# tatsuya-ogawa/GaussianSplattingMlx

Hardware: AMD Instinct MI355X
Metric: train views/sec (full step: fwd + L1/DSSIM loss + bwd + Adam + densify/prune at the reference cadence), Lego 800x800 300k Gaussians (higher is better)
Workload: dtype f32

## Files before the change

### gaussiansplattingmlx_amd/_lib.py

```python
from __future__ import annotations

import ctypes as C
import os

HERE = os.path.dirname(os.path.abspath(__file__))
LIB_PATH = os.environ.get("GSPLAT_LIB", os.path.join(HERE, "libgsplat_hip.so"))

GS_OK = 0
STATUS = {1: "GS_ERR_INVALID_ARG", 2: "GS_ERR_SIZE_MISMATCH", 3: "GS_ERR_WORKSPACE_OVERFLOW", 4: "GS_ERR_HIP",
          5: "GS_ERR_NO_FORWARD", 6: "GS_ERR_NO_DEVICE", 7: "GS_ERR_IO", 8: "GS_ERR_COMM", 9: "GS_ERR_REPLICA_MISMATCH"}
GS_ERR_REPLICA_MISMATCH = 9


class GsplatError(RuntimeError):
    def __init__(self, code, msg):
        super().__init__(f"{STATUS.get(code, code)}: {msg}")
        self.code = code


class gs_camera(C.Structure):
    _fields_ = [("view", C.c_float * 16), ("proj", C.c_float * 16), ("cam_center", C.c_float * 3),
                ("fov_x", C.c_float), ("fov_y", C.c_float), ("focal_x", C.c_float), ("focal_y", C.c_float)]


# ... 26 lines not shown

class gs_adc_params(C.Structure):
    _fields_ = [(n, C.c_float) for n in ("grad_threshold", "percent_dense", "min_opacity", "max_screen_size", "prune_world",
                                         "scene_extent")]


GS_DEPTH_ACCUMULATED, GS_DEPTH_EXPECTED, GS_DEPTH_DISPARITY = 0, 1, 2
GS_DP_ALLREDUCE, GS_DP_SH_COMPRESSED = 0, 1
GS_DP_UNIQUE_ID_BYTES = 128

_vp = C.c_void_p
_SIGS = {
    "gs_dp_unique_id": (C.c_int, [_vp]),
    "gs_dp_init": (C.c_int, [_vp, _vp, C.c_int, C.c_int]),
    "gs_dp_attach": (C.c_int, [_vp, _vp, C.c_int, C.c_int]),
    "gs_dp_shutdown": (C.c_int, [_vp]),
    "gs_dp_info": (C.c_int, [_vp, C.POINTER(C.c_int), C.POINTER(C.c_int)]),
    "gs_dp_step": (C.c_int, [_vp, C.c_int, C.POINTER(gs_dp_step_args)]),
    "gs_dp_allreduce_sum": (C.c_int, [_vp, _vp, C.c_longlong]),
    "gs_dp_check_overflow": (C.c_int, [_vp, C.POINTER(C.c_int), C.POINTER(C.c_longlong)]),
    "gs_dp_exchange_timing": (C.c_int, [_vp, C.c_int]),
    "gs_dp_exchange_read": (C.c_int, [_vp, _vp, C.POINTER(C.c_int), C.POINTER(C.c_int)]),
    "gs_abi_version": (C.c_int, []),
    "gs_ctx_create": (C.c_int, [C.c_int] * 7 + [C.POINTER(_vp)]),
    "gs_ctx_destroy": (C.c_int, [_vp]),
    "gs_ctx_set_stream": (C.c_int, [_vp, _vp]),
    "gs_ctx_reserve": (C.c_int, [_vp, C.c_int, C.c_longlong]),
    "gs_workspace_bytes": (C.c_size_t, [_vp]),
    "gs_sync": (C.c_int, [_vp]),
    "gs_overflow_pending": (C.c_int, [_vp, C.POINTER(C.c_uint32)]),
    "gs_wait": (C.c_int, [_vp]),
    "gs_last_error": (C.c_char_p, [_vp]),
    "gs_projection_forward": (C.c_int, [_vp, C.c_int, C.c_int] + [_vp] * 4 + [C.POINTER(gs_camera)] + [_vp] * 8),
    "gs_projection_backward": (C.c_int, [_vp, C.c_int, C.c_int] + [_vp] * 4 + [C.POINTER(gs_camera)] + [_vp] * 10),
    "gs_tile_bin": (C.c_int, [_vp, C.c_int] + [_vp] * 4),
    "gs_tile_bin_cut": (C.c_int, [_vp, C.c_int] + [_vp] * 5),
    "gs_tile_bin_info": (C.c_int, [_vp, C.POINTER(C.c_uint32), C.POINTER(C.c_uint32)]),
    "gs_tile_bin_views": (C.c_int, [_vp, C.POINTER(_vp), C.POINTER(_vp), C.POINTER(_vp)]),
    "gs_tile_bin_export": (C.c_int, [_vp, _vp, _vp, _vp]),
    "gs_build_packed_tile_indices": (C.c_int, [_vp, C.c_uint32, _vp]),
    "gs_pack_gaussians": (C.c_int, [_vp, C.c_int] + [_vp] * 6),
    "gs_blend_forward": (C.c_int, [_vp, C.c_int] + [_vp] * 5),
    "gs_blend_backward": (C.c_int, [_vp, C.c_int] + [_vp] * 9),
    "gs_blend_contrib": (C.c_int, [_vp, C.c_int] + [_vp] * 3),
    "gs_render_contrib": (C.c_int, [_vp, _vp, _vp]),
    "gs_contrib_actions": (C.c_int, [_vp, C.c_int, _vp, C.c_float, _vp, _vp]),
    "gs_ssim_window": (C.c_int, [C.c_int, C.c_float, _vp]),
    "gs_ssim_forward": (C.c_int, [_vp] + [C.c_int] * 4 + [_vp] * 9),
    "gs_ssim_backward": (C.c_int, [_vp] + [C.c_int] * 4 + [_vp] * 11),
    "gs_render_forward": (C.c_int, [_vp, C.c_int, C.c_int] + [_vp] * 6 + [C.POINTER(gs_camera)] + [_vp] * 4),
    "gs_render_backward": (C.c_int, [_vp] + [_vp] * 9),
    "gs_render_backward_dp": (C.c_int, [_vp] + [_vp] * 8),
    "gs_render_backward_adam": (C.c_int, [_vp] * 7 + [C.c_longlong, _vp, C.c_float, C.c_float, C.c_float, C.c_float]),
    "gs_render_backward_dp_begin": (C.c_int, [_vp] * 5),
    "gs_render_backward_dp_finish": (C.c_int, [_vp] * 5),
    "gs_render_backward_dp_finish_geom": (C.c_int, [_vp] * 6),
    "gs_render_backward_dp_geom": (C.c_int, [_vp] * 10),
    "gs_sh_grad_from_views_adam_dir": (C.c_int, [_vp, C.c_int, C.c_int, C.c_int] + [_vp] * 9 + [C.c_longlong] + [C.c_float] * 6 + [_vp]),
    "gs_adam_step_add": (C.c_int, [_vp, C.c_longlong] + [_vp] * 4 + [C.c_int, _vp, _vp] + [C.c_float] * 4 + [_vp, C.c_longlong]),
    "gs_sh_grad_from_views": (C.c_int, [_vp, C.c_int, C.c_int, C.c_int] + [_vp] * 5),
    "gs_accum_grad_norm": (C.c_int, [_vp, C.c_int, _vp, _vp, _vp]),
    "gs_classify_gaussians": (C.c_int, [_vp, C.c_int, _vp, C.c_float, _vp, C.c_int, _vp, C.c_float, C.c_float,
                                        C.c_float, C.c_int, _vp, _vp]),
    "gs_densify_offsets": (C.c_int, [_vp, C.c_int, _vp, _vp, _vp, _vp]),
    "gs_build_densify_output_map": (C.c_int, [_vp, C.c_int, _vp, _vp, C.c_int, _vp, _vp]),
    "gs_densify_gather": (C.c_int, [_vp, C.c_int, C.c_int] + [_vp] * 15),
    "gs_densify_plan": (C.c_int, [_vp, C.c_int, _vp, _vp, _vp]),
    "gs_densify_plan_read": (C.c_int, [_vp, C.c_int, _vp, C.POINTER(C.c_int)]),
    "gs_build_densify_output_map_planned": (C.c_int, [_vp, C.c_int, _vp, _vp, C.c_int, _vp, _vp]),
    "gs_densify_gather_planned": (C.c_int, [_vp, C.c_int, C.c_int] + [_vp] * 8 + [C.c_ulonglong] + [_vp] * 6),
    "gs_densify_gather_planned_packed": (C.c_int, [_vp, C.c_int, C.c_int] + [_vp] * 8 + [C.c_ulonglong, _vp, C.POINTER(C.c_int)]),
    "gs_densify_noise": (C.c_int, [_vp, C.c_ulonglong, C.c_int, _vp]),
    "gs_ply_write": (C.c_int, [_vp, C.c_char_p, C.c_int, C.c_int] + [_vp] * 6),
    "gs_ply_probe": (C.c_int, [_vp, C.c_char_p, _vp, _vp, _vp]),
    "gs_ply_load": (C.c_int, [_vp, C.c_char_p, C.c_int, C.c_int] + [_vp] * 6),
    "gs_ply_pack_rows": (C.c_int, [_vp, C.c_int, C.c_int] + [_vp] * 7),
    "gs_set_block_work_buffer": (C.c_int, [_vp, _vp]),
    "gs_view_hint_words": (C.c_int, [_vp, C.POINTER(C.c_int)]),
    "gs_set_view_hints": (C.c_int, [_vp, _vp, C.c_int]),
    "gs_set_depth_cuts": (C.c_int, [_vp, C.c_int]),
    "gs_clear_depth_cuts": (C.c_int, [_vp, _vp, C.c_int]),
    "gs_forward_missed": (C.c_int, [_vp, C.POINTER(C.c_int)]),
    "gs_cut_stats": (C.c_int, [_vp, C.POINTER(C.c_uint32)]),
    "gs_set_grad_norm_accum": (C.c_int, [_vp, _vp]),
    "gs_block_count": (C.c_int, [_vp, _vp]),
    "gs_copy_block_work": (C.c_int, [_vp, _vp]),
    "gs_dist_topk": (C.c_int, [_vp, C.c_int, C.c_int, C.c_int, C.c_int, _vp, _vp]),
    "gs_sh_grad_from_views_adam": (C.c_int, [_vp, C.c_int, C.c_int, C.c_int] + [_vp] * 8 + [C.c_longlong] + [C.c_float] * 6),
    "gs_loss_target_cache_floats": (C.c_int, [_vp, C.POINTER(C.c_longlong)]),
    "gs_set_loss_target_cache": (C.c_int, [_vp, _vp, C.c_int]),
    "gs_set_loss_mask": (C.c_int, [_vp, _vp]),
    "gs_loss_forward_backward": (C.c_int, [_vp] + [_vp] * 5 + [C.c_float, C.c_float] + [_vp] * 3),
    "gs_depth_loss": (C.c_int, [_vp, C.POINTER(gs_depth_loss_params)] + [_vp] * 7),
    "gs_depth_normalize": (C.c_int, [_vp, C.c_longlong, _vp, _vp, C.c_float, _vp]),
    "gs_image_metrics": (C.c_int, [_vp, C.c_int, C.c_int] + [_vp] * 4),
    "gs_colour_moments": (C.c_int, [_vp, C.c_longlong] + [_vp] * 4),
    "gs_adam_step": (C.c_int, [_vp, C.c_longlong] + [_vp] * 4 + [C.c_int, _vp, _vp] + [C.c_float] * 4),
    "gs_profile_enable": (C.c_int, [_vp, C.c_uint]),
    "gs_profile_read": (C.c_int, [_vp, _vp, _vp]),
    "gs_copy_last_contrib": (C.c_int, [_vp, _vp]),
    "gs_last_stats": (C.c_int, [_vp, C.POINTER(C.c_uint32)]),
    "gs_ctx_set_tuning": (C.c_int, [_vp, C.c_int, C.c_longlong]),
    "gs_copy_overflow_flag": (C.c_int, [_vp, _vp]),
    "gs_set_update_gate": (C.c_int, [_vp, _vp]),
    "gs_set_overflow_rider": (C.c_int, [_vp, _vp]),
    "gs_set_pose_correction": (C.c_int, [_vp, _vp, _vp]),
# ... 11 lines not shown
    "gs_get_absgrad": (C.c_int, [_vp, C.c_int, _vp]),
    "gs_set_adc_stats": (C.c_int, [_vp, _vp, _vp, _vp]),
    "gs_adc_accumulate": (C.c_int, [_vp, C.c_int, _vp, _vp, C.c_int, _vp, _vp, _vp]),
    "gs_adc_classify": (C.c_int, [_vp, C.c_int] + [_vp] * 4 + [C.c_int, _vp, C.POINTER(gs_adc_params), C.c_int, C.c_int, _vp, _vp]),
    "gs_adc_gather": (C.c_int, [_vp, C.c_int, C.c_int] + [_vp] * 9 + [C.c_int] + [_vp] * 6),
    "gs_adc_gather_moments": (C.c_int, [_vp, C.c_int, C.c_int, _vp, _vp, _vp, C.POINTER(_vp), C.POINTER(_vp)]),
    "gs_adc_reset_opacity": (C.c_int, [_vp, C.c_int, _vp, _vp, _vp, C.c_float]),
    "gs_set_sparse_adam": (C.c_int, [_vp, C.c_int]),
    "gs_get_visibility": (C.c_int, [_vp, C.c_int, _vp]),
    "gs_adam_step_visible": (C.c_int, [_vp, C.c_longlong] + [_vp] * 4 + [C.c_int, _vp, _vp, _vp] + [C.c_float] * 4 + [C.c_int, _vp]),
    "gs_set_filter3d_cameras": (C.c_int, [_vp, C.c_int, _vp]),
    "gs_compute_filter3d": (C.c_int, [_vp, C.c_int, _vp, _vp]),
    "gs_set_filter3d": (C.c_int, [_vp, _vp]),
    "gs_filter3d_bake": (C.c_int, [_vp, C.c_int] + [_vp] * 5),
    "gs_undistort": (C.c_int, [_vp, C.POINTER(gs_lens)] + [C.c_int] * 6 + [_vp, _vp, _vp]),
    "gs_undistort_fisheye": (C.c_int, [_vp, C.POINTER(gs_fisheye_lens)] + [C.c_int] * 6 + [_vp, _vp, _vp]),
    "gs_set_mcmc": (C.c_int, [_vp, _vp]),
    "gs_mcmc_regularizer_grad": (C.c_int, [_vp, C.c_int] + [_vp] * 5),
    "gs_mcmc_inject_noise": (C.c_int, [_vp, C.c_int] + [_vp] * 4 + [C.c_float, _vp]),
    "gs_mcmc_random": (C.c_int, [_vp, C.c_ulonglong, C.c_int, C.c_int, C.c_int, _vp, _vp, _vp]),
    "gs_mcmc_relocate": (C.c_int, [_vp, C.c_int, C.c_int] + [_vp] * 11),
    "gs_mcmc_grow": (C.c_int, [_vp, C.c_int, C.c_int, C.c_int] + [_vp] * 11),
    "gs_set_gathered_gate": (C.c_int, [_vp, C.c_longlong, C.c_int, _vp]),
    "gs_set_gate_seen": (C.c_int, [_vp, _vp]),
    "gs_dp_cc_floats": (C.c_longlong, [C.c_int]),
    "gs_dp_check_replicas": (C.c_int, [_vp, C.c_int, _vp, C.c_longlong]),
    "gs_dp_check_replicas_begin": (C.c_int, [_vp, C.c_int, _vp, C.c_longlong]),
    "gs_dp_check_replicas_end": (C.c_int, [_vp]),
    "gs_dp_check_plan": (C.c_int, [_vp, C.POINTER(C.c_longlong), C.c_int]),
}

_lib = None


def load():
    global _lib
    if _lib is not None:
        return _lib
    if not os.path.exists(LIB_PATH):
        raise ImportError(f"{LIB_PATH} is missing: run `python -m gaussiansplattingmlx_amd.build` "
                          "(or __graft_entry__.build()). There is no CPU fallback.")
    import torch
    lib = C.CDLL(LIB_PATH)
    for name, (res, args) in _SIGS.items():
        fn = getattr(lib, name)
        fn.restype = res
        fn.argtypes = args
    _lib = lib
    return lib


TUNE_FWD_WAVES_PER_SIMD, TUNE_BWD_WAVES_PER_CU, TUNE_FWD_QUADRANTS, TUNE_OP_FWD_PPL, TUNE_OP_BWD_PPL, \
    TUNE_FWD_TRACE_BUFFER, TUNE_DEPTH_GRADIENT, TUNE_WIDE_TILE_SORT, TUNE_HOST_OVERFLOW_ERRORS, TUNE_SPLITTER_DEPTH_SORT, \
    TUNE_COLOUR_RIDERS, TUNE_FWD_QUEUES, TUNE_FWD_FOUR_WAVES, TUNE_FWD_FOLD_TEST_SCALE, TUNE_POISON_CHECKPOINTS, TUNE_RENDER_ONLY, TUNE_FWD_PAIR, TUNE_FWD_SLOW_SLOT, TUNE_TRIM_RECTS = range(19)


def exported_symbols():
    return list(_SIGS)


def make_camera(view, proj, camCenter, fovX, fovY, focalX, focalY) -> gs_camera:
    import numpy as np
    cam = gs_camera()
    v = np.asarray(view, dtype=np.float32).reshape(16)
    p = np.asarray(proj, dtype=np.float32).reshape(16)
    cc = np.asarray(camCenter, dtype=np.float32).reshape(3)
    for i in range(16):
        cam.view[i] = float(v[i])
        cam.proj[i] = float(p[i])
    for i in range(3):
        cam.cam_center[i] = float(cc[i])
    cam.fov_x, cam.fov_y, cam.focal_x, cam.focal_y = float(fovX), float(fovY), float(focalX), float(focalY)
    return cam
```

### gaussiansplattingmlx_amd/csrc/api.hip

```cpp
#include <math.h>
#include <stdlib.h>
#include <stdio.h>
#include <string.h>

#include "gs_ctx.h"
#include <vector>

using namespace gs;

namespace {

int fail(gs_ctx* c, int code, const std::string& msg)
{
    if (c) c->err = msg;
    return code;
}

template <class T>
int dev_alloc(gs_ctx* c, T** p, size_t count)
{
    *p = nullptr;
    if (count == 0) count = 1;
    GS_HIP_CHECK(c, hipMalloc((void**)p, count * sizeof(T)));
    c->ws_bytes += count * sizeof(T);
    return GS_OK;
}

template <class T>
void dev_free(T*& p)
{
    if (p) (void)hipFree(p);
    p = nullptr;
}

void free_gaussian_ws(gs_ctx* c)
{
    dev_free(c->packed12); dev_free(c->gradAcc16);
    dev_free(c->depthKey[0]); dev_free(c->depthKey[1]); dev_free(c->depthVal[0]); dev_free(c->depthVal[1]);
    dev_free(c->tilesTouched); dev_free(c->tileRect); dev_free(c->tilePieces); dev_free(c->waveSeg); dev_free(c->scanPrefix); dev_free(c->scanTmp); dev_free(c->blockSums);
    dev_free(c->visPerBlock); dev_free(c->dropPerBlock);
    dev_free(c->bucketId);
    dev_free(c->densifyTiles);
    c->densifyTileCap = 0;
}

void free_pair_ws(gs_ctx* c)
{
    dev_free(c->pairKey[0]); dev_free(c->pairKey[1]); dev_free(c->pairVal[0]); dev_free(c->pairVal[1]);
    dev_free(c->segSlot); dev_free(c->itemBlock); dev_free(c->itemRow);
}

int ensure_arena(gs_ctx* c)
{
    if (!c->fast16 || c->capM <= 0) return GS_OK;
    long long want = (c->pairsReserved || c->reserving) ? c->capM / 80 : c->segCap * 4;
    if (want < 65536) want = 65536;
    if (want > c->segCap * 4) want = c->segCap * 4;
    if (want < c->qslotWanted) want = c->qslotWanted;
    if (want <= c->qslotCap) return GS_OK;
    GS_HIP_CHECK(c, hipStreamSynchronize(c->stream));
    if (c->segState) { c->ws_bytes -= (size_t)c->qslotCap * 5 * 64 * sizeof(float); dev_free(c->segState); }
    const int rc = dev_alloc(c, &c->segState, (size_t)want * 5 * 64);
    if (rc) { c->qslotCap = 0; return rc; }
    c->qslotCap = want;
    c->fwd.valid = false;
    return GS_OK;
}

int ensure_capacity(gs_ctx* c, int N, long long M)
{
    bool grewN = false, grewM = false;
    if (N > c->capN) {
        GS_HIP_CHECK(c, hipStreamSynchronize(c->stream));
        free_gaussian_ws(c);
        const size_t n = (size_t)N;
        int rc;
        if ((rc = dev_alloc(c, &c->packed12, n * 12))) return rc;
        if ((rc = dev_alloc(c, &c->gradAcc16, n * 16))) return rc;
        for (int i = 0; i < 2; i++) {
            if ((rc = dev_alloc(c, &c->depthKey[i], n))) return rc;
            if ((rc = dev_alloc(c, &c->depthVal[i], n))) return rc;
        }
        if ((rc = dev_alloc(c, &c->tilesTouched, n))) return rc;
        if ((rc = dev_alloc(c, &c->tileRect, n))) return rc;
        if ((rc = dev_alloc(c, &c->tilePieces, n))) return rc;
        if ((rc = dev_alloc(c, &c->waveSeg, (n / 64 + 8) * GS_EXPAND_SLICES))) return rc;
        if ((rc = dev_alloc(c, &c->scanPrefix, (n / 64 + 16) * GS_EXPAND_SLICES))) return rc;
        if ((rc = dev_alloc(c, &c->scanTmp, (n / 64 + 16) * GS_EXPAND_SLICES / 1024 + 8))) return rc;
        const size_t nb = n / GS_SCAN_BLOCK + 2;
        if ((rc = dev_alloc(c, &c->blockSums, nb))) return rc;
        if ((rc = dev_alloc(c, &c->visPerBlock, n / 128 + 2))) return rc;
        dev_free(c->dropPerBlock);
        if ((rc = dev_alloc(c, &c->dropPerBlock, n / 128 + 2))) return rc;
        if ((rc = dev_alloc(c, &c->bucketId, n + 16))) return rc;
        c->capN = N;
        grewN = true;
// ... 256 lines not shown
{
    if (!c->poseDelta && !c->fwd.poseDelta) return GS_OK;
    return fail(c, GS_ERR_INVALID_ARG, std::string(who) + ": a pose correction is set (single-device steps only)");
}

int refuse_absgrad(gs_ctx* c, const char* who)
{
    if (!c->absgrad) return GS_OK;
    return fail(c, GS_ERR_INVALID_ARG, std::string(who) + ": absgrad is on (gs_set_absgrad): only gs_render_backward and "
                                       "gs_render_backward_adam accumulate the absolute sums");
}

int refuse_adc_stats(gs_ctx* c, const char* who)
{
    if (!c->adcGradSum) return GS_OK;
    return fail(c, GS_ERR_INVALID_ARG, std::string(who) + ": the ADC statistic is set (gs_set_adc_stats): only gs_render_backward and "
                                       "gs_render_backward_adam accumulate it");
}

int refuse_sparse_adam(gs_ctx* c, const char* who)
{
    if (!c->sparseAdam) return GS_OK;
    return fail(c, GS_ERR_INVALID_ARG, std::string(who) + ": sparse Adam is on (gs_set_sparse_adam): single-device steps through "
                                       "gs_render_backward_adam or gs_adam_step_visible only");
}

int refuse_filter3d(gs_ctx* c, const char* who)
{
    if (!c->filter3d && !(c->fwd.valid && c->fwd.filter3d)) return GS_OK;
    return fail(c, GS_ERR_INVALID_ARG, std::string(who) + ": a 3-D filter is set (single-device steps only)");
}

int refuse_fisheye(gs_ctx* c, const char* who)
{
    if (!c->fisheye && !(c->fwd.valid && c->fwd.fisheye)) return GS_OK;
    return fail(c, GS_ERR_INVALID_ARG, std::string(who) + ": the fisheye camera model is set (gs_set_camera_model; pinhole cameras only)");
}

int forward_in_arena(gs_ctx* c, const char* who, const float* params_base, long long n_arena)
{
    const int N = c->fwd.N, K = c->fwd.K;
    const float* lo = params_base;
    const float* hi = params_base + n_arena;
    auto inside = [&](const float* p, long long n) { return n == 0 || (p >= lo && p + n <= hi); };
    if (inside(c->fwd.xyz, 3LL * N) && inside(c->fwd.fdc, 3LL * N) && inside(c->fwd.frest, 3LL * (K - 1) * N) &&
        inside(c->fwd.scales, 3LL * N) && inside(c->fwd.rot, 4LL * N) && inside(c->fwd.opacity, N))
        return GS_OK;
    return fail(c, GS_ERR_SIZE_MISMATCH, std::string(who) + ": the forward's tensors do not lie in the arena");
}

}

#pragma GCC visibility push(default)
extern "C" {

int gs_abi_version(void) { return GSPLAT_ABI_VERSION; }

int gs_ctx_create(int device, int W, int H, int tile_w, int tile_h, int sh_degree, int white_bg, gs_ctx** out)
{
    if (!out) return GS_ERR_INVALID_ARG;
    *out = nullptr;
    if (W <= 0 || H <= 0 || tile_w <= 0 || tile_h <= 0 || sh_degree < 0 || sh_degree > 4) return GS_ERR_INVALID_ARG;
    int ndev = 0;
    if (hipGetDeviceCount(&ndev) != hipSuccess || ndev <= 0 || device < 0 || device >= ndev) return GS_ERR_NO_DEVICE;
    gs_ctx* c = new gs_ctx();
    c->device = device;
    c->W = W; c->H = H; c->tileW = tile_w; c->tileH = tile_h;
    c->gridW = (W + tile_w - 1) / tile_w; c->gridH = (H + tile_h - 1) / tile_h;
    c->T = c->gridW * c->gridH;
    c->degree = sh_degree; c->whiteBg = white_bg ? 1 : 0;
    c->bg.mode = c->whiteBg ? GS_BG_WHITE : GS_BG_BLACK;
    c->fast16 = (tile_w % 16 == 0) && (tile_h % 16 == 0);
    c->blocksX = gs_div_up(W, 16); c->blocksY = gs_div_up(H, 16);
    c->real.tileW = tile_w; c->real.tileH = tile_h; c->real.gridW = c->gridW; c->real.gridH = c->gridH; c->real.T = c->T;
    c->real.fast16 = c->fast16;
    {
        const char* e = getenv("GSPLAT_BLOCK_LISTS");
        const int nbx = gs_div_up(tile_w, 16), nby = gs_div_up(tile_h, 16);
        if (!c->fast16 && !(e && atoi(e) == 0) && (long long)c->gridW * nbx <= 65535 && (long long)c->gridH * nby <= 65535) {
            c->virt.nbx = nbx; c->virt.nby = nby; c->virt.tw = tile_w; c->virt.th = tile_h;
            c->tileW = 16; c->tileH = 16;
            c->gridW *= nbx; c->gridH *= nby;
            c->T = c->gridW * c->gridH;
            c->fast16 = true;
            c->blocksX = c->gridW; c->blocksY = c->gridH;
        }
    }
    if (const char* e = getenv("GSPLAT_COLOUR_RIDERS")) c->colourRiders = atoi(e);
    if (const char* e = getenv("GSPLAT_FWD_WIDE")) c->fwdWide = atoi(e) < 0 ? -1 : atoi(e) != 0;
    if (const char* e = getenv("GSPLAT_FWD_QUEUES")) { const int q = atoi(e); if (q >= 1 && q <= (int)GS_QUEUES && !(q & (q - 1))) c->fwdQueues = q; }
    if (const char* e = getenv("GSPLAT_RIDER_SHARES")) {
        int vals[GS_RIDE_HOSTS + 1], n = 0;
        for (const char* q = e; *q && n <= GS_RIDE_HOSTS; n++) {
            vals[n] = atoi(q);
            while (*q && *q != ',') q++;
            if (*q == ',') q++;
        }
        if (n == GS_RIDE_HOSTS) for (int i = 0; i < GS_RIDE_HOSTS; i++) c->riderShare[i] = vals[i];
        else fprintf(stderr, "gsplat: GSPLAT_RIDER_SHARES needs %d comma-separated values (got %s): ignored\n", GS_RIDE_HOSTS, e);
    }
    if (c->gridW > 65535 || c->gridH > 65535) { delete c; return GS_ERR_INVALID_ARG; }
    int bits = 1;
    while ((1LL << bits) < c->T) bits++;
    c->tileBits = bits;
    for (bits = 1; (1LL << bits) < c->real.T; bits++) {}
    c->real.tileBits = bits;
// ... 375 lines not shown
    if (N < 0 || K < 1 || !cam) return fail(c, GS_ERR_INVALID_ARG, "gs_render_forward: bad N/K/cam");
    if ((c->degree + 1) * (c->degree + 1) > K) return fail(c, GS_ERR_SIZE_MISMATCH, "K smaller than (degree+1)^2");
    if (!out_color || !out_alpha) return fail(c, GS_ERR_INVALID_ARG, "gs_render_forward: null output");
    if (N > 0 && (!xyz || !features_dc || (K > 1 && !features_rest) || !scales || !rotation || !opacity))
        return fail(c, GS_ERR_INVALID_ARG, "gs_render_forward: null parameter tensor");
    if (c->fisheye && c->poseDelta)
        return fail(c, GS_ERR_INVALID_ARG, "gs_render_forward: the fisheye camera model has no pose refinement (gs_set_pose_correction is set)");
    if (c->fisheye && c->filter3d)
        return fail(c, GS_ERR_INVALID_ARG, "gs_render_forward: the fisheye camera model has no 3-D filter (gs_set_filter3d is set)");
    c->fwd.valid = false;
    c->visN = -1;
    const bool keepRadii = c->sparseAdam || c->adcGradSum != nullptr;
    if (keepRadii && N > c->visCap) {
        GS_HIP_CHECK(c, hipStreamSynchronize(c->stream));
        if (c->visMask) c->ws_bytes -= (size_t)c->visCap * (sizeof(unsigned char) + sizeof(float));
        dev_free(c->visMask); dev_free(c->visRadii);
        c->visCap = 0;
        const int cap = N > c->capN ? N : c->capN;
        if (const int arc = dev_alloc(c, &c->visMask, (size_t)cap)) return arc;
        if (const int arc = dev_alloc(c, &c->visRadii, (size_t)cap)) {
            c->ws_bytes -= (size_t)cap * sizeof(unsigned char);
            dev_free(c->visMask);
            return arc;
        }
        c->visCap = cap;
    }
    if (keepRadii && !radii) radii = c->visRadii;
    c->binIsBlockLists = c->virt.nbx != 0;
    const bool reserved = c->pairsReserved && c->capN >= N;
    if (reserved) { const int orc = deferred_overflow(c); if (orc) return orc; }
    if (c->fwd.cutsActive && !c->fwd.missChecked) GS_HIP_CHECK(c, hipEventSynchronize(c->fwdDone));
    c->fwd.missed = false;
    c->fwd.bwdPrepared = false;
    c->fwd.arenaOverflow = false;
    c->fwd.cutStore = c->cutStore;
    c->fwd.cutsActive = c->cutStore != nullptr && c->allowCuts && N > 0;
    c->fwd.missChecked = !c->fwd.cutsActive;
    if (c->fwd.cutsActive) c->missHost[0] = 0;
    const CamParams cp = make_cam(cam, c->W, c->H);
    if (c->poseDelta) {
        const long long need = pose_partials_floats(N);
        if (need > c->posePartialsCap) {
            GS_HIP_CHECK(c, hipStreamSynchronize(c->stream));
            dev_free(c->posePartials);
            c->posePartialsCap = 0;
            if (const int arc = dev_alloc(c, &c->posePartials, (size_t)need)) return arc;
            c->posePartialsCap = need;
        }
        if (const int prc = launch_pose_camera(c, cp, c->poseDelta)) return prc;
    }
    c->segBaseWanted = c->fast16 && N > 0;
    c->segBaseDone = false;
    c->fwdPairNow = c->fast16 && blend_forward_v2_pair_decide(c);
    int rc = bin_with_capacity(c, N, reserved, !c->fast16, [&]() {
        return launch_projection_fused_forward(c, N, K, xyz, features_dc, features_rest, scales, rotation, opacity, cp,
                                               radii);
    });
    c->segBaseWanted = false;
    if (rc) { c->rider.on = false; return rc; }
    if (c->rider.on && c->rider.next < c->rider.total) {
        GsStageTimer t(c, GS_STAGE_PROJ_FWD, true);
        if ((rc = launch_colour_rest(c))) return rc;
    }
    c->rider.on = false;
    {
        GsStageTimer t(c, GS_STAGE_BLEND_FWD);
        rc = c->fast16 ? launch_blend_forward_v2(c, out_color, out_depth, out_alpha)
                       : launch_blend_forward(c, c->bg, out_color, out_depth, out_alpha, c->lastContrib);
        if (rc) return rc;
    }
    if (c->fwd.cutsActive) GS_HIP_CHECK(c, hipEventRecord(c->fwdDone, c->stream));
    c->fwd.valid = true;
    c->absgradN = -1;
    c->fwd.blendBackwardDone = false;
    c->fwd.consumed = false;
    c->fwd.blockWork = c->blockWork;
    c->fwd.N = N; c->fwd.K = K;
    c->fwd.xyz = xyz; c->fwd.fdc = features_dc; c->fwd.frest = features_rest; c->fwd.scales = scales;
    c->fwd.rot = rotation; c->fwd.opacity = opacity;
    c->fwd.outColor = out_color; c->fwd.outDepth = out_depth; c->fwd.outAlpha = out_alpha;
    c->fwd.cam = cp;
    c->fwd.poseDelta = c->poseDelta;
    c->fwd.poseGrad = c->poseGrad;
    c->fwd.antialias = c->antialias;
    c->fwd.fisheye = c->fisheye;
    c->fwd.bg = c->bg;
    c->fwd.filter3d = c->filter3d;
    c->fwd.radii = keepRadii ? radii : nullptr;
    if (c->sparseAdam) c->visN = N;
    return GS_OK;
}

int gs_set_sparse_adam(gs_ctx* c, int enable)
{
    if (!c) return GS_ERR_INVALID_ARG;
    if (enable != 0 && enable != 1) return fail(c, GS_ERR_INVALID_ARG, "gs_set_sparse_adam: enable is 0 or 1");
    if (enable && c->mcmcOn)
        return fail(c, GS_ERR_INVALID_ARG, "gs_set_sparse_adam: the MCMC strategy is set (its noise and regularisers act on every Gaussian)");
    if (enable && c->filter3d) return fail(c, GS_ERR_INVALID_ARG, "gs_set_sparse_adam: a 3-D filter is set (gs_set_filter3d)");
    c->sparseAdam = enable == 1;
    return GS_OK;
}

int gs_get_visibility(gs_ctx* c, int N, unsigned char* out)
{
    if (!c) return GS_ERR_INVALID_ARG;
    if (c->visN < 0)
// ... 451 lines not shown
    if ((long long)W * H > 0 && (!grid || !in || !out)) return fail(c, GS_ERR_INVALID_ARG, "gs_apply_bilateral_grid: null buffer");
    return launch_bilateral_apply(c, W, H, grid, grid_w, grid_h, grid_l, in, out);
}

int gs_render_backward(gs_ctx* c, const float* cot_color, const float* cot_depth, const float* cot_alpha,
                       float* grad_xyz, float* grad_features_dc, float* grad_features_rest, float* grad_scales,
                       float* grad_rotation, float* grad_opacity)
{
    if (!c) return GS_ERR_INVALID_ARG;
    { const int prc = backward_preflight(c, "gs_render_backward", cot_depth != nullptr); if (prc) return prc; }
    const int N = c->fwd.N, K = c->fwd.K;
    if (!cot_color) return fail(c, GS_ERR_INVALID_ARG, "gs_render_backward: null cot_color");
    if (N > 0 && (!grad_xyz || !grad_features_dc || (K > 1 && !grad_features_rest) || !grad_scales || !grad_rotation ||
                  !grad_opacity))
        return fail(c, GS_ERR_INVALID_ARG, "gs_render_backward: null gradient buffer");
    if (const int rc = blend_backward_of_forward(c, cot_color, cot_depth, cot_alpha, c->absgrad, nullptr)) return rc;
    AbsgradScope noNorm(c);
    GsStageTimer t(c, GS_STAGE_PROJ_BWD);
    return launch_projection_fused_backward(c, grad_xyz, grad_features_dc, grad_features_rest, grad_scales, grad_rotation, grad_opacity);
}

int gs_render_contrib(gs_ctx* c, float* max_w, float* sum_w)
{
    if (!c) return GS_ERR_INVALID_ARG;
    { const int prc = backward_preflight(c, "gs_render_contrib", false); if (prc) return prc; }
    if (!max_w && !sum_w) return fail(c, GS_ERR_INVALID_ARG, "gs_render_contrib: null buffer (one of max_w, sum_w at least)");
    return launch_blend_contrib(c, max_w, sum_w);
}

int gs_contrib_actions(gs_ctx* c, int N, const float* score, float threshold, int* actions, int* output_counts)
{
    if (!c) return GS_ERR_INVALID_ARG;
    if (N < 0 || !(threshold == threshold) || (N > 0 && (!score || !actions || !output_counts)))
        return fail(c, GS_ERR_INVALID_ARG, "gs_contrib_actions: bad arguments");
    return launch_contrib_actions(c, N, score, threshold, actions, output_counts);
}

int gs_render_backward_adam(gs_ctx* c, const float* cot_color, const float* cot_depth, const float* cot_alpha,
                            float* params_base, float* m_base, float* v_base, long long n_arena, const float lr[6],
                            float beta1, float beta2, float eps, float grad_scale)
{
    if (!c) return GS_ERR_INVALID_ARG;
    { const int prc = backward_preflight(c, "gs_render_backward_adam", cot_depth != nullptr); if (prc) return prc; }
    const int N = c->fwd.N, K = c->fwd.K;
    if (!cot_color || !lr || n_arena < 0 || (N > 0 && (!params_base || !m_base || !v_base)))
        return fail(c, GS_ERR_INVALID_ARG, "gs_render_backward_adam: null buffer");
    if (const int rc = forward_in_arena(c, "gs_render_backward_adam", params_base, n_arena)) return rc;
    if (c->sparseAdam && (c->visN != N || c->fwd.filter3d))
        return fail(c, GS_ERR_NO_FORWARD, "gs_render_backward_adam: sparse Adam is on, but the forward was not made under it "
                                          "(gs_set_sparse_adam comes before gs_render_forward)");
    if (const int rc = blend_backward_of_forward(c, cot_color, cot_depth, cot_alpha, c->absgrad, c->adamGate)) return rc;
    c->fwd.consumed = true;
    AbsgradScope noNorm(c);
    GsStageTimer t(c, GS_STAGE_PROJ_BWD);
    return launch_projection_fused_backward_adam(c, params_base, m_base, v_base, lr, beta1, beta2, eps, grad_scale);
}

int gs_render_backward_dp_begin(gs_ctx* c, const float* cot_color, const float* cot_depth, const float* cot_alpha,
                                float* color_cot)
{
    if (!c) return GS_ERR_INVALID_ARG;
    if (const int rc = refuse_pose_correction(c, "gs_render_backward_dp_begin")) return rc;
    if (const int rc = refuse_filter3d(c, "gs_render_backward_dp_begin")) return rc;
    if (const int rc = refuse_fisheye(c, "gs_render_backward_dp_begin")) return rc;
    if (const int rc = refuse_sparse_adam(c, "gs_render_backward_dp_begin")) return rc;
    if (const int rc = refuse_absgrad(c, "gs_render_backward_dp_begin")) return rc;
    if (const int rc = refuse_adc_stats(c, "gs_render_backward_dp_begin")) return rc;
    { const int prc = backward_preflight(c, "gs_render_backward_dp_begin", cot_depth != nullptr); if (prc) return prc; }
    const int N = c->fwd.N;
    if (!cot_color || (N > 0 && !color_cot)) return fail(c, GS_ERR_INVALID_ARG, "gs_render_backward_dp_begin: null buffer");
    if (const int rc = blend_backward_of_forward(c, cot_color, cot_depth, cot_alpha)) return rc;
    c->fwd.blendBackwardDone = true;
    GsStageTimer t(c, GS_STAGE_PROJ_BWD);
    return launch_color_cot(c, N, color_cot);
}

int gs_render_backward_dp_finish(gs_ctx* c, float* grad_xyz, float* grad_scales, float* grad_rotation, float* grad_opacity)
{
    if (!c) return GS_ERR_INVALID_ARG;
    if (const int rc = refuse_pose_correction(c, "gs_render_backward_dp_finish")) return rc;
    if (const int rc = refuse_filter3d(c, "gs_render_backward_dp_finish")) return rc;
    if (const int rc = refuse_fisheye(c, "gs_render_backward_dp_finish")) return rc;
    if (const int rc = refuse_sparse_adam(c, "gs_render_backward_dp_finish")) return rc;
    if (!c->fwd.valid || !c->fwd.blendBackwardDone)
        return fail(c, GS_ERR_NO_FORWARD, "gs_render_backward_dp_finish: no gs_render_backward_dp_begin on this context");
    const int N = c->fwd.N, K = c->fwd.K;
    if (N > 0 && (!grad_xyz || !grad_scales || !grad_rotation || !grad_opacity))
        return fail(c, GS_ERR_INVALID_ARG, "gs_render_backward_dp_finish: null gradient buffer");
    c->fwd.blendBackwardDone = false;
    GsStageTimer t(c, GS_STAGE_PROJ_BWD);
    return launch_projection_fused_backward(c, grad_xyz, nullptr, nullptr, grad_scales, grad_rotation, grad_opacity, true);
}

int gs_render_backward_dp_finish_geom(gs_ctx* c, float* grad_xyz, float* grad_scales, float* grad_rotation, float* grad_opacity,
                                      float* xyz_own)
{
    if (!c) return GS_ERR_INVALID_ARG;
    if (const int rc = refuse_pose_correction(c, "gs_render_backward_dp_finish_geom")) return rc;
    if (const int rc = refuse_filter3d(c, "gs_render_backward_dp_finish_geom")) return rc;
    if (const int rc = refuse_fisheye(c, "gs_render_backward_dp_finish_geom")) return rc;
    if (const int rc = refuse_sparse_adam(c, "gs_render_backward_dp_finish_geom")) return rc;
    if (!c->fwd.valid || !c->fwd.blendBackwardDone)
        return fail(c, GS_ERR_NO_FORWARD, "gs_render_backward_dp_finish_geom: no gs_render_backward_dp_begin on this context");
    const int N = c->fwd.N;
    if (N > 0 && (!grad_xyz || !grad_scales || !grad_rotation || !grad_opacity || !xyz_own))
        return fail(c, GS_ERR_INVALID_ARG, "gs_render_backward_dp_finish_geom: null buffer");
    c->fwd.blendBackwardDone = false;
    GsStageTimer t(c, GS_STAGE_PROJ_BWD);
// ... 262 lines not shown
    if (!c->fwd.valid || !c->fwd.cutsActive) return GS_OK;
    if (!c->fwd.missChecked) return fail(c, GS_ERR_INVALID_ARG, "gs_cut_stats: ask gs_forward_missed first");
    out[0] = c->missHost[1]; out[1] = c->missHost[2];
    return GS_OK;
}

int gs_ctx_set_tuning(gs_ctx* c, int knob, long long value)
{
    if (!c) return GS_ERR_INVALID_ARG;
    switch (knob) {
    case GS_TUNE_FWD_WAVES_PER_SIMD:
        if (value < 1 || value > 16) return fail(c, GS_ERR_INVALID_ARG, "gs_ctx_set_tuning: forward waves per SIMD must be 1..16");
        c->fwdWavesPerSimd = (int)value; return GS_OK;
    case GS_TUNE_BWD_WAVES_PER_CU:
        if (value < 1 || value > 64) return fail(c, GS_ERR_INVALID_ARG, "gs_ctx_set_tuning: backward waves per CU must be 1..64");
        c->bwdWavesPerCu = (int)value; return GS_OK;
    case GS_TUNE_FWD_QUADRANTS:
        c->fwdQuadrants = value != 0; return GS_OK;
    case GS_TUNE_FWD_QUEUES:
        if (value < 1 || value > (long long)GS_QUEUES || (value & (value - 1))) return fail(c, GS_ERR_INVALID_ARG, "gs_ctx_set_tuning: forward queues must be 1, 2, 4 or 8");
        c->fwdQueues = (int)value; return GS_OK;
    case GS_TUNE_FWD_FOUR_WAVES:
        c->fwdWide = value < 0 ? -1 : (value != 0); return GS_OK;
    case GS_TUNE_OP_FWD_PPL:
    case GS_TUNE_OP_BWD_PPL:
        if (value != 1 && value != 2 && value != 4) return fail(c, GS_ERR_INVALID_ARG, "gs_ctx_set_tuning: pixels per lane must be 1, 2 or 4");
        (knob == GS_TUNE_OP_FWD_PPL ? c->opFwdPpl : c->opBwdPpl) = (int)value; return GS_OK;
    case GS_TUNE_WIDE_TILE_SORT:
        c->wideTileSort = value != 0; return GS_OK;
    case GS_TUNE_DEPTH_GRADIENT:
        c->depthGradient = value != 0; return GS_OK;
    case GS_TUNE_HOST_OVERFLOW_ERRORS:
        c->hostOverflowErrors = value != 0; return GS_OK;
    case GS_TUNE_SPLITTER_DEPTH_SORT:
        c->splitterSort = value > 0; c->haveSplitters = false; return GS_OK;
    case GS_TUNE_COLOUR_RIDERS:
        c->colourRiders = (int)value; return GS_OK;
    case GS_TUNE_FWD_FOLD_TEST_SCALE:
        if (value < 1 || value > 1000) return fail(c, GS_ERR_INVALID_ARG, "gs_ctx_set_tuning: fold test scale is in permille, 1..1000");
        c->fwdFoldScale = (float)value / 1000.0f; return GS_OK;
    case GS_TUNE_POISON_CHECKPOINTS:
        c->poisonCheckpoints = value != 0; return GS_OK;
    case GS_TUNE_RENDER_ONLY:
        c->renderOnly = value != 0; return GS_OK;
    case GS_TUNE_FWD_SLOW_SLOT:
        if (value < 1 || value > 16) return fail(c, GS_ERR_INVALID_ARG, "gs_ctx_set_tuning: the first slow wave slot must be 1..16 (16 = none)");
        c->fwdSlowSlot = (int)value; return GS_OK;
    case GS_TUNE_FWD_PAIR:
        if (value < -1 || value > 16) return fail(c, GS_ERR_INVALID_ARG, "gs_ctx_set_tuning: forward pair workgroups per CU must be -1 (by list depth), 0..16");
        c->fwdPair = (int)value; return GS_OK;
    case GS_TUNE_TRIM_RECTS:
        if (value < 0 || value > 2) return fail(c, GS_ERR_INVALID_ARG, "gs_ctx_set_tuning: trim rects is 0 (the reference's squares), 1 (cut by the ellipse's box) or 2 (and into four row groups)");
        c->trimRects = value != 0; c->rowGroups = value == 2; return GS_OK;
    case GS_TUNE_FWD_TRACE_BUFFER:
        c->fwdTrace = reinterpret_cast<unsigned long long*>((uintptr_t)value); return GS_OK;
    default:
        return fail(c, GS_ERR_INVALID_ARG, "gs_ctx_set_tuning: unknown knob");
    }
}

int gs_copy_overflow_flag(gs_ctx* c, uint32_t* out)
{
    if (!c || !out) return GS_ERR_INVALID_ARG;
    hipLaunchKernelGGL(copy_word_kernel, dim3(1), dim3(1), 0, c->stream, c->counters + GS_CNT_OVERFLOW, out);
    GS_HIP_CHECK(c, hipGetLastError());
    return GS_OK;
}

int gs_set_update_gate(gs_ctx* c, const uint32_t* gate)
{
    if (!c) return GS_ERR_INVALID_ARG;
    c->adamGate = gate ? gate : c->counters + GS_CNT_OVERFLOW;
    return GS_OK;
}

int gs_set_overflow_rider(gs_ctx* c, float* dst)
{
    if (!c) return GS_ERR_INVALID_ARG;
    c->overflowRider = dst;
    return GS_OK;
}

int gs_set_gathered_gate(gs_ctx* c, long long block_floats, int count, uint32_t* reduced_out)
{
    if (!c) return GS_ERR_INVALID_ARG;
    if (block_floats < 0 || (block_floats > 0 && (count < 1 || count > 16)))
        return fail(c, GS_ERR_INVALID_ARG, "gs_set_gathered_gate: bad block size / count (1..16 blocks)");
    c->ccBlockFloats = block_floats;
    c->ccBlockCount = block_floats > 0 ? count : 0;
    c->gatheredGateOut = block_floats > 0 ? reduced_out : nullptr;
    return GS_OK;
}

int gs_set_gate_seen(gs_ctx* c, uint32_t* seen)
{
    if (!c) return GS_ERR_INVALID_ARG;
    c->gateSeen = seen;
    return GS_OK;
}

int gs_set_grad_norm_accum(gs_ctx* c, float* accum)
{
    if (!c) return GS_ERR_INVALID_ARG;
    c->gradNormAccum = accum;
    return GS_OK;
}
// ... 313 lines not shown
```

### gaussiansplattingmlx_amd/csrc/gs_ctx.h

```cpp
#pragma once
#include <hip/hip_runtime.h>
#include <stdint.h>

#include <string>
#include <vector>

#include "../../include/gsplat.h"
#include "gs_math.h"

enum {
    GS_CNT_M = 0,
    GS_CNT_OVERFLOW = 1,
    GS_CNT_MREQ = 2,
    GS_CNT_B = 3,
    GS_CNT_NVIS = 4,
    GS_CNT_CONTRIB_LO = 5,
    GS_CNT_CONTRIB_HI = 6,
    GS_CNT_ITEMS = 9,
    GS_CNT_CUT_DROPPED = 12,
    GS_CNT_QSLOTS = 16,
    GS_CNT_COUNT = 24
};

constexpr uint32_t GS_QUEUES = 8;
// ... 25 lines not shown
struct GsBackground {
    int mode = GS_BG_BLACK;
    float r = 0.0f, g = 0.0f, b = 0.0f;
};
#if defined(__HIPCC__)
__device__ __forceinline__ void gs_bg_terms(const GsBackground& bg, float T, float& t0, float& t1, float& t2)
{
    if (bg.mode == GS_BG_COLOUR) { t0 = __fmul_rn(T, bg.r); t1 = __fmul_rn(T, bg.g); t2 = __fmul_rn(T, bg.b); }
    else t0 = t1 = t2 = bg.mode ? T : 0.0f;
}
__device__ __forceinline__ float gs_bg_cot(const GsBackground& bg, float gx, float gy, float gz)
{
    if (bg.mode == GS_BG_COLOUR) return fmaf(gx, bg.r, fmaf(gy, bg.g, __fmul_rn(gz, bg.b)));
    return bg.mode ? (gx + gy + gz) : 0.0f;
}
#endif

struct GsDp;

struct GsColourRider {
    const float* xyz;
    const float* fdc;
    const float* frest;
    float* packed12;
    const uint32_t* tilesTouched;
    float cam[3];
    int N, degree;
    int unit0, units;
};
enum { GS_RIDE_SS_HIST = 0, GS_RIDE_SS_SCATTER, GS_RIDE_WIDE_TILE, GS_RIDE_HOSTS };
struct GsRiderState {
    bool on = false;
    GsColourRider args = {};
    int next = 0, total = 0;
};

struct GsVirtGeom {
    int nbx = 0, nby = 0;
    int tw = 0, th = 0;
};
__device__ __forceinline__ void gs_block_pixels(const GsVirtGeom& g, int bx, int by, int W, int H, int& X0, int& Y0, int& XL, int& YL)
{
    if (g.nbx == 0) { X0 = bx * 16; Y0 = by * 16; XL = W; YL = H; return; }
    const int tx = bx / g.nbx, ix = bx - tx * g.nbx, ty = by / g.nby, iy = by - ty * g.nby;
    X0 = tx * g.tw + ix * 16; Y0 = ty * g.th + iy * 16;
    XL = min(W, min(X0 + 16, (tx + 1) * g.tw)); YL = min(H, min(Y0 + 16, (ty + 1) * g.th));
}
constexpr int GS_F3D_CAM_FLOATS = 16;
constexpr int GS_CUT_SUPER = 4;
struct GsCutCoarse {
    const uint32_t* superCut = nullptr;
    int superW = 0;
    uint32_t* dropPerBlock = nullptr;
};
struct GsRealGeom {
    int tileW = 16, tileH = 16, gridW = 0, gridH = 0, T = 0, tileBits = 1;
    bool fast16 = false;
};

struct gs_ctx {
    int device = 0;
    GsDp* dp = nullptr;
    hipStream_t stream = nullptr;
    hipStream_t own_stream = nullptr;
    int W = 0, H = 0, tileW = 16, tileH = 16, gridW = 0, gridH = 0, T = 0, degree = 0, whiteBg = 0;
    int tileBits = 1;
    GsBackground bg;
    bool fast16 = false;
    GsVirtGeom virt;
    GsRealGeom real;
    bool binIsBlockLists = false;
    int blocksX = 0, blocksY = 0;
    std::string err;

    int capN = 0;
    long long capM = 0;
    bool pairsReserved = false;
    bool reserving = false;
    size_t ws_bytes = 0;

    float* packed12 = nullptr;
    float* gradAcc16 = nullptr;
    uint32_t* depthKey[2] = {nullptr, nullptr};
    uint32_t* depthVal[2] = {nullptr, nullptr};
    uint32_t* tilesTouched = nullptr;
    uint4* tilePieces = nullptr;
    bool piecesValid = false;
    ushort4* tileRect = nullptr;
    uint32_t* blockSums = nullptr;
    uint32_t* visPerBlock = nullptr;
    int visBlocks = 0;
    uint32_t* pairKey[2] = {nullptr, nullptr};
    uint32_t* pairVal[2] = {nullptr, nullptr};
    uint32_t* hist = nullptr;
    uint32_t* rowTotal = nullptr;
    uint16_t* wideCnt = nullptr;
    uint32_t* wideChunk = nullptr;
    uint32_t* wideTotal = nullptr;
    uint2* sortBits = nullptr;
    uint32_t* sortSplit[2] = {nullptr, nullptr};
    int splitCur = 0;
    bool haveSplitters = false;
    unsigned char* bucketId = nullptr;
    uint32_t* bucketStart = nullptr;
    int colourRiders = 1;
    GsRiderState rider;
    int riderShare[GS_RIDE_HOSTS] = {200, 500, 300};
    int splitterSort = 1;
    int nbCap = 0;
    bool superCutReady = false;
    uint32_t* dropPerBlock = nullptr;
    int dropBlocks = 0;
    uint32_t* superCut = nullptr;
    uint32_t* tileRanges = nullptr;
    uint32_t* tileCounts = nullptr;
    uint32_t* blockWork = nullptr;
    uint32_t* blockWorkOwn = nullptr;
    uint32_t* blockOrder = nullptr;
    uint32_t* fwdQueue = nullptr;
    uint32_t* bwdQueue = nullptr;
    uint32_t* cutStore = nullptr;
    bool allowCuts = true;
    const uint32_t* opCuts = nullptr;
    unsigned long long* scanTmp = nullptr;
    unsigned long long* scanPrefix = nullptr;
    uint2* waveSeg = nullptr;
    uint32_t* missHost = nullptr;
    uint32_t* missDev = nullptr;
    hipEvent_t fwdDone = nullptr;
    const uint32_t* workHint = nullptr;
    const float* poseDelta = nullptr;
    float* poseGrad = nullptr;
    gs::CamParams* poseCam = nullptr;
    float* posePartials = nullptr;
    long long posePartialsCap = 0;
    const float* expoM = nullptr;
    float* expoGrad = nullptr;
    float* correctedImage = nullptr;
    double* expoPartials = nullptr;
    const float* bgGrid = nullptr;
    float* bgGrad = nullptr;
    int bgW = 0, bgH = 0, bgL = 0;
    float bgTv = 0.0f;
    int bgChunks = 0, bgChunksW = 0, bgChunksH = 0;
    float* bgPartials = nullptr;
    long long bgPartialsCap = 0;
    bool antialias = false;
    bool fisheye = false;
    bool absgrad = false;
    int absgradN = -1;
    bool sparseAdam = false;
    unsigned char* visMask = nullptr;
    float* visRadii = nullptr;
    int visCap = 0;
    int visN = -1;
    float* adcGradSum = nullptr;
    float* adcCount = nullptr;
    float* adcMaxRadius = nullptr;
    const float* filter3d = nullptr;
// ... 122 lines not shown
static inline bool gs_small_depth_sort(long long n) { return gs_div_up(n, GS_SORT_THREADS * GS_SMALL_SORT_ITEMS) <= GS_SMALL_SORT_BLOCKS; }

struct GsStageTimer {
    gs_ctx* c;
    int slot = -1;
    GsStageTimer(gs_ctx* ctx, int stage, bool extra = false) : c(ctx)
    {
        if (!((c->profMask >> stage) & 1u)) return;
        if (c->profUsed == c->profPool.size()) {
            if (c->profPool.size() >= 16384) return;
            gs_ctx::ProfEvent e;
            if (hipEventCreate(&e.a) != hipSuccess) return;
            if (hipEventCreate(&e.b) != hipSuccess) { (void)hipEventDestroy(e.a); return; }
            c->profPool.push_back(e);
        }
        slot = (int)c->profUsed++;
        c->profPool[slot].stage = stage;
        c->profPool[slot].extra = extra;
        (void)hipEventRecord(c->profPool[slot].a, c->stream);
    }
    ~GsStageTimer()
    {
        if (slot >= 0) (void)hipEventRecord(c->profPool[slot].b, c->stream);
    }
};

namespace gs {

int refuse_pose_correction(gs_ctx* c, const char* who);
int refuse_fisheye(gs_ctx* c, const char* who);
int refuse_filter3d(gs_ctx* c, const char* who);
int refuse_absgrad(gs_ctx* c, const char* who);
int refuse_sparse_adam(gs_ctx* c, const char* who);
int refuse_adc_stats(gs_ctx* c, const char* who);
int forward_in_arena(gs_ctx* c, const char* who, const float* params_base, long long n_arena);

CamParams make_cam(const gs_camera* cam, int W, int H);

int launch_projection_forward(gs_ctx* c, int N, int K, const float* scales, const float* rot, const float* means3d,
                              const float* shs, const CamParams& cam, float* means2d, float* depths, float* color,
                              float* cov2d, float* conic, float* radii, float* rectMin, float* rectMax);
int launch_projection_backward(gs_ctx* c, int N, int K, const float* scales, const float* rot, const float* means3d,
                               const float* shs, const CamParams& cam, const float* cotDepths,
                               const float* cotMeans2d, const float* cotCov2d, const float* cotColor,
                               const float* cotConic, float* gScales, float* gRot, float* gMeans, float* gShs,
                               float* gCam);
int launch_projection_fused_forward(gs_ctx* c, int N, int K, const float* xyz, const float* fdc, const float* frest,
                                    const float* scales, const float* rot, const float* opacity,
                                    const CamParams& cam, float* radii);
int launch_projection_fused_backward(gs_ctx* c, float* gXyz, float* gFdc, float* gFrest, float* gScales, float* gRot, float* gOpacity,
                                     bool emitColorCot = false);
int launch_projection_fused_backward_adam(gs_ctx* c, const float* pBase, float* mBase, float* vBase, const float lr[6], float b1,
                                          float b2, float eps, float gscale);
int launch_vis_mask(gs_ctx* c, int N, const float* radii);
bool depth_sort_takes_splitters(const gs_ctx* c, int N);
int launch_pose_camera(gs_ctx* c, const gs::CamParams& host, const float* delta);
int launch_pose_grad(gs_ctx* c, int N);
long long pose_partials_floats(int N);
int launch_exposure_apply(gs_ctx* c, long long n, const float* M, const float* in, float* out);
int launch_exposure_backward(gs_ctx* c, long long n, const float* M, const float* render, float* cot, double* partials,
                             float* grad);
long long exposure_partials_doubles();
bool bilateral_shape_ok(int gw, int gh, int gl);
int bilateral_chunks(int W, int H, int gw, int gh);
long long bilateral_partials_floats(int gw, int gh, int gl, int nch);
int launch_bilateral_apply(gs_ctx* c, int W, int H, const float* G, int gw, int gh, int gl, const float* in, float* out);
int launch_bilateral_backward(gs_ctx* c, int W, int H, const float* G, int gw, int gh, int gl, int nch, float tvWeight,
                              const float* render, float* cot, float* partials, float* grad);
int launch_composite_target(gs_ctx* c, long long n, const float* rgb, const float* alpha, const float bg[3], float* out);
long long depth_loss_ws_doubles();
int launch_depth_loss(gs_ctx* c, int mode, float lambda, float alphaMin, float scale, float offset, const float* depth,
                      const float* alpha, const float* target, const unsigned char* mask, float* loss, float* cotDepth,
                      float* cotAlpha);
int launch_depth_normalize(gs_ctx* c, long long n, const float* depth, const float* alpha, float alphaMin, float* out);
long long metrics_ws_doubles(int H, int W);
int launch_image_metrics(gs_ctx* c, int H, int W, const float* render, const float* target, const unsigned char* mask, double* out);
int launch_colour_moments(gs_ctx* c, long long n, const float* render, const float* target, const unsigned char* mask, double* out);
int launch_filter3d_width(gs_ctx* c, int N, const float* xyz, float* filter);
int launch_filter3d_bake(gs_ctx* c, int N, const float* scalesRaw, const float* opacityRaw, const float* filter, float* outScales,
                         float* outOpacity);
int launch_undistort(gs_ctx* c, const gs_lens& lens, int srcW, int srcH, int dstW, int dstH, int channels, int mode, const void* src,
                     void* dst, unsigned char* valid);
int launch_undistort_fisheye(gs_ctx* c, const gs_fisheye_lens& lens, int srcW, int srcH, int dstW, int dstH, int channels, int mode, const void* src,
                     void* dst, unsigned char* valid);
int launch_colour_rest(gs_ctx* c);
int launch_color_cot(gs_ctx* c, int N, float* out);
int launch_sh_grad_from_views(gs_ctx* c, int N, int K, int R, const float* xyz, const float* mgAll,
                              const float* camCentersHost, float* gFdc, float* gFrest);
int launch_sh_grad_from_views_adam(gs_ctx* c, int N, int K, int R, const float* xyz, const float* mgAll,
                                   const float* camCentersHost, const float* fdcParam, const float* frestParam,
                                   const float* pBase, float* mBase, float* vBase, float lrDc, float lrRest, float b1,
                                   float b2, float eps, float gscale);
int launch_projection_geom_backward(gs_ctx* c, float* gXyz, float* gScales, float* gRot, float* gOpacity, float* xyzOwn,
                                    float* colorCot = nullptr);
int launch_sh_views_dir_adam(gs_ctx* c, int N, int K, int R, const float* xyz, const float* mgAll, const float* camCentersHost,
                             const float* const* ownXyzHost, const float* fdcParam, const float* frestParam, const float* pBase,
                             float* mBase, float* vBase, float lrDc, float lrRest, float b1, float b2, float eps, float gscale,
                             float* xyzAdd);
int launch_pack11_to_12(gs_ctx* c, int N, const float* packed11);
int launch_pack_gaussians(gs_ctx* c, int N, const float* means2d, const float* conic, const float* color,
                          const float* opacity, const float* depths, float* packed11);

int launch_bin_prep(gs_ctx* c, int N, const float* rectMin, const float* rectMax, const float* radii,
                    const float* depths);
int launch_binning(gs_ctx* c, int N, bool wantPlain);
int ensure_plain_sorted(gs_ctx* c);
// ... 98 lines not shown
```

### gaussiansplattingmlx_amd/csrc/gs_proj_fwd_kernel.h

```cpp
constexpr bool proj_fwd_form_exists(bool TWO_PHASE, bool COLOUR, bool SELF, bool POSE, bool F3D = false, bool FISHEYE = false)
{
    return (COLOUR ? !SELF : (TWO_PHASE && !POSE)) && (!FISHEYE || (!POSE && !F3D));
}

template <bool TWO_PHASE, bool COLOUR, bool SELF, bool AA, bool F3D, bool POSE, bool FISHEYE = false>
__global__ __launch_bounds__(PROJ_FUSED_THREADS) void proj_fwd_fused_kernel(
    int N, int K, int degree, CamParams hostCam, int tileW, int tileH, int gridW, int gridH,
    const float* __restrict__ xyz, const float* __restrict__ fdc, const float* __restrict__ frest,
    const float* __restrict__ scalesRaw, const float* __restrict__ rotRaw, const float* __restrict__ opacityRaw,
    float* __restrict__ packed12, float* __restrict__ radiiOut, ushort4* __restrict__ tileRect,
    uint32_t* __restrict__ tilesTouched, uint32_t* __restrict__ depthKey, uint32_t* __restrict__ depthVal,
    uint32_t* __restrict__ visPerBlock, uint32_t* __restrict__ counters, int flags, ColourRider self,
    GsVirtGeom vg, GsCutCoarse cc, uint4* __restrict__ tilePieces, const float* __restrict__ filter3d,
    const CamParams* __restrict__ dcam)
{
    static_assert(proj_fwd_form_exists(TWO_PHASE, COLOUR, SELF, POSE, F3D, FISHEYE), "no such form of the fused projection forward");
    CamParams posed;
    if constexpr (POSE) posed = *dcam;
    const CamParams& cam = POSE ? posed : hostCam;
    const int noKeyForUntouched = flags & 1;
    const bool trimRects = (flags & 2) && !vg.nbx && tileW == 16 && tileH == 16;
    extern __shared__ float shLds[];
    __shared__ uint32_t sDropped;
    if (cc.superCut) {
// ... 84 lines not shown
        }
        uint32_t gate = 0u;
        if (COLOUR) {
            c0 += 0.5f; c1 += 0.5f; c2 += 0.5f;
            gate = colour_gate(c0, c1, c2);
        }

        float4* out = reinterpret_cast<float4*>(packed12 + (size_t)p * 12);
        out[0] = make_float4(o.sx, o.sy, o.conic[0], o.conic[1]);
        out[1] = make_float4(o.conic[2], o.conic[3], c0, c1);
        out[2] = make_float4(c2, opacity, o.depth, __uint_as_float(gate));
        if (radiiOut) radiiOut[p] = o.radius;

        uint32_t touched = 0;
        ushort4 tr = make_ushort4(0, 0, 0, 0);
        uint32_t pc[4] = {0u, 0u, 0u, 0u};
        if (o.radius > 0.0f) {
            int x0, y0, x1, y1;
            if (vg.nbx)
                block_rect_of_splat(o.rect, o.sx, o.sy, o.cov2d[0], o.cov2d[3], vg.nbx, vg.nby, vg.tw, vg.th, gridW / vg.nbx,
                                    gridH / vg.nby, (int)cam.W, (int)cam.H, x0, y0, x1, y1);
            else if (trimRects)
                block_rect_of_splat(o.rect, o.sx, o.sy, o.cov2d[0], o.cov2d[3], 1, 1, 16, 16, gridW, gridH, (int)cam.W, (int)cam.H,
                                    x0, y0, x1, y1);
            else
                tile_rect(o.rect[0], o.rect[1], o.rect[2], o.rect[3], tileW, tileH, gridW, gridH, x0, y0, x1, y1);
            touched = (uint32_t)((x1 - x0) * (y1 - y0));
            if (trimRects && tilePieces && touched)
                touched = rect_row_groups4(o.sx, o.sy, o.cov2d[0], o.cov2d[1], o.cov2d[3], x0, y0, x1, y1, (int)cam.H, pc);
            tr = make_ushort4((unsigned short)x0, (unsigned short)y0, (unsigned short)x1, (unsigned short)y1);
            visible = true;
            if (cc.superCut && touched) {
                const uint32_t key = __float_as_uint(o.depth);
                bool reach = false;
                const int sx1 = (x1 - 1) / GS_CUT_SUPER, sy1 = (y1 - 1) / GS_CUT_SUPER;
                for (int sy = y0 / GS_CUT_SUPER; sy <= sy1 && !reach; sy++)
                    for (int sx = x0 / GS_CUT_SUPER; sx <= sx1; sx++)
                        if (key <= 0xFFFFFFFFu - cc.superCut[sy * cc.superW + sx]) { reach = true; break; }
                if (!reach) { atomicAdd(&sDropped, touched); touched = 0; tr = make_ushort4(0, 0, 0, 0); pc[0] = pc[1] = pc[2] = pc[3] = 0u; }
            }
        }
        tileRect[p] = tr;
        if (trimRects && tilePieces) tilePieces[p] = make_uint4(pc[0], pc[1], pc[2], pc[3]);
        tilesTouched[p] = touched;
        myTouched = touched;
        depthKey[p] = (touched || !noKeyForUntouched) ? __float_as_uint(o.depth) : GS_SORT_NO_KEY;
        depthVal[p] = (uint32_t)p;
    }
    const int nvis = __syncthreads_count(visible);
    if (threadIdx.x == 0) visPerBlock[blockIdx.x] = (uint32_t)nvis;
    if (cc.superCut && threadIdx.x == 0) cc.dropPerBlock[blockIdx.x] = sDropped;
    if (SELF) colour_rider_wave(self, blockIdx.x * (PROJ_FUSED_THREADS / 64) + wv, shLds + wv * 64 * GS_RIDER_ROW, lane, (int)myTouched);
}
```

### gaussiansplattingmlx_amd/csrc/projection.hip

```cpp
#include <type_traits>

#include "gs_ctx.h"
#include "gs_mcmc.h"
#include "gs_rider.h"

namespace gs {

constexpr int PROJ_THREADS = 256;

CamParams make_cam(const gs_camera* cam, int W, int H)
{
    CamParams p;
    for (int i = 0; i < 16; i++) { p.V[i] = cam->view[i]; p.P[i] = cam->proj[i]; }
    for (int i = 0; i < 3; i++) p.cam[i] = cam->cam_center[i];
    p.fovX = cam->fov_x; p.fovY = cam->fov_y; p.focalX = cam->focal_x; p.focalY = cam->focal_y;
    p.limX = tanf(cam->fov_x * 0.5f) * 1.3f;
    p.limY = tanf(cam->fov_y * 0.5f) * 1.3f;
    p.W = (float)W; p.H = (float)H;
    return p;
}

template <bool FISHEYE>
__device__ __forceinline__ void proj_fwd_op_body(
    int N, int K, int degree, const CamParams& cam, const float* __restrict__ scales, const float* __restrict__ rot,
// ... 333 lines not shown
            if constexpr (SPARSE) {
                float4 mz = make_float4(0.f, 0.f, 0.f, 0.f), vz = mz;
                if (vis4(e)) { mz = M4[e]; vz = V4[e]; }
                m[b] = mz; v[b] = vz;
            } else {
                m[b] = M4[e]; v[b] = V4[e];
            }
        }
    };
    auto update = [&](int k, float4 (&m)[B], float4 (&v)[B]) {
#pragma unroll
        for (int b = 0; b < B; b++) {
            const int e = lane + 64 * (k * B + b);
            bool on = e < total4;
            if constexpr (SPARSE) on = on && vis4(e);
            if (on) {
                float4& p = pp[k * B + b];
                adam_step(adam, grad_at(4 * e), lr, p.x, m[b].x, v[b].x);
                adam_step(adam, grad_at(4 * e + 1), lr, p.y, m[b].y, v[b].y);
                adam_step(adam, grad_at(4 * e + 2), lr, p.z, m[b].z, v[b].z);
                adam_step(adam, grad_at(4 * e + 3), lr, p.w, m[b].w, v[b].w);
                P4[e] = p; M4[e] = m[b]; V4[e] = v[b];
            }
        }
    };
#pragma unroll
    for (int k = 0; k < D - 1 && k < NB; k++) load(k, mm[k % D], vv[k % D]);
#pragma unroll
    for (int k = 0; k < NB; k++) {
        if (k + D - 1 < NB) load(k + D - 1, mm[(k + D - 1) % D], vv[(k + D - 1) % D]);
        update(k, mm[k % D], vv[k % D]);
    }
}

__device__ __forceinline__ void drop_nonfinite_row(float4& g0, float4& g1, float4& g2)
{
#ifdef GS_KEEP_NONFINITE_ROWS
    return;
#endif
    auto fin = [](float v) { return (v - v) == 0.0f; };
    if (!(fin(g0.x) && fin(g0.y) && fin(g0.z) && fin(g0.w) && fin(g1.x) && fin(g1.y) && fin(g1.z) && fin(g1.w) && fin(g2.x) &&
          fin(g2.y) && fin(g2.z))) {
        g0 = make_float4(0.f, 0.f, 0.f, 0.f); g1 = g0; g2 = g0;
    }
}

__device__ __forceinline__ float wave_sum_xor(float v)
{
#pragma unroll
    for (int o = 32; o >= 1; o >>= 1) v += __shfl_xor(v, o, 64);
    return v;
}

template <int MODE, bool POSE, bool AA = false, bool MCMC = false, bool F3D = false, bool SPARSE = false, bool FISHEYE = false>
__device__ __forceinline__ void proj_bwd_fused_body(
    int N, int K, int degree, const CamParams& cam, const float* xyz, const float* fdc,
    const float* frest, const float* scalesRaw, const float* rotRaw,
    const float* opacityRaw, const float* __restrict__ gradAcc16, float* gXyz,
    float* gFdc, float* gFrest, float* gScales, float* gRot,
    float* gOpacity, float* __restrict__ gradNormAccum, AdamFuse adam, float* __restrict__ posePartials,
    McmcFuse mc = McmcFuse{}, const float* __restrict__ filter3d = nullptr, const unsigned char* __restrict__ visMask = nullptr)
{
    constexpr bool EMIT_MG = MODE == 1, ADAM = MODE == 2;
    extern __shared__ float shLds[];
    const uint32_t gateWord = ADAM ? *adam.gate : 0u;
    const int p = blockIdx.x * PROJ_FUSED_THREADS + threadIdx.x;
    if (MODE == 0 && adam.rider && p == 0) *adam.rider = *adam.ovf ? 1.0f : 0.0f;
    const int lane = threadIdx.x & 63, wv = threadIdx.x >> 6;
    bool myVis = true;
    unsigned long long visBits = ~0ull;
    if constexpr (SPARSE) {
        myVis = p < N && visMask[p] != 0;
        visBits = __ballot(myVis);
        if (visBits == 0ull) {
            if constexpr (POSE) {
                if (lane < 16) posePartials[16 * ((size_t)blockIdx.x * (PROJ_FUSED_THREADS / 64) + wv) + lane] = 0.f;
            }
            return;
        }
    }
    const int L = (K - 1) * 3;
    float* myRows = shLds + wv * 64 * (L + 1);
    const int row0 = blockIdx.x * PROJ_FUSED_THREADS + wv * 64;
    const int rows = min(64, N - row0);
    float4 keptRows[SH_ROWS_MAX4];
    const int total4 = (rows * L) >> 2;
    const bool kept = ADAM && rows > 0 && L > 0 && (L & 3) == 0 && total4 <= 64 * SH_ROWS_MAX4 &&
                      (((size_t)(frest - adam.pBase) + (size_t)row0 * L) & 3) == 0;
    if (kept) {
        sh_rows_load4(frest + (size_t)row0 * L, total4, 0, lane, keptRows);
        sh_rows_to_lds4(myRows, total4, L, 0, lane, keptRows);
    } else if (rows > 0 && L > 0) sh_rows_in(myRows, frest + (size_t)row0 * L, rows, L, lane);
    float pose[POSE ? 15 : 1];
    if constexpr (POSE) {
#pragma unroll
        for (int j = 0; j < 15; j++) pose[j] = 0.f;
    }
    if (p < N) {
    const float4* ga = reinterpret_cast<const float4*>(gradAcc16 + (size_t)p * 16);
    float4 g0 = ga[0], g1 = ga[1], g2 = ga[2];
    drop_nonfinite_row(g0, g1, g2);
    const float cm[2] = {g0.x, g0.y};
    const float ccon[4] = {g0.z, g0.w, g1.x, g1.y};
    const float ccol[3] = {g1.z, g1.w, g2.x};
    const float cotOpacity = g2.y, cotDepth = g2.z;
    const float ccov[4] = {0.f, 0.f, 0.f, 0.f};

    const float m[3] = {xyz[3 * p], xyz[3 * p + 1], xyz[3 * p + 2]};
    const float sr[3] = {scalesRaw[3 * p], scalesRaw[3 * p + 1], scalesRaw[3 * p + 2]};
    const float s[3] = {expf(sr[0]), expf(sr[1]), expf(sr[2])};
    const float rr[4] = {rotRaw[4 * p], rotRaw[4 * p + 1], rotRaw[4 * p + 2], rotRaw[4 * p + 3]};
    const float n2 = rr[0] * rr[0] + rr[1] * rr[1] + rr[2] * rr[2] + rr[3] * rr[3];
    const float nrm = sqrtf(n2);
    const float den = nrm + 1e-8f;
    const float q[4] = {rr[0] / den, rr[1] / den, rr[2] / den, rr[3] / den};

// ... 87 lines not shown
    if constexpr (F3D) {
        const float sgF = 1.0f / (1.0f + expf(-opr));
        filter3d_activate<true>(s, f3dF, se, g.ds, cotOpacity * sgF * (AA ? aaRho : 1.0f) * f3dKappa);
    }
#pragma unroll
    for (int a = 0; a < 3; a++) {
        const float v = F3D ? g.ds[a] : g.ds[a] * s[a];
        if (ADAM) sg_[3 + a] = v; else gScales[3 * p + a] = v;
    }
    const float dot = g.dq[0] * rr[0] + g.dq[1] * rr[1] + g.dq[2] * rr[2] + g.dq[3] * rr[3];
    const float dn = -dot / (den * den);
    const float dn2 = dn * 0.5f / nrm;
#pragma unroll
    for (int a = 0; a < 4; a++) {
        const float v = g.dq[a] / den + 2.0f * rr[a] * dn2;
        if (ADAM) sg_[6 + a] = v; else gRot[4 * p + a] = v;
    }
    const float sg = 1.0f / (1.0f + expf(-opr));
    const float gop = (F3D ? (AA ? cotOpacity * f3dKappa * aaRho : cotOpacity * f3dKappa) : AA ? cotOpacity * aaRho : cotOpacity) * sg * (1.0f - sg);
    if (ADAM) sg_[10] = gop; else gOpacity[p] = gop;
    if constexpr (MCMC) {
        sg_[10] = sg_[10] + mc.oCoef * mcmc_sigmoid_slope(opr);
#pragma unroll
        for (int a = 0; a < 3; a++) sg_[3 + a] = sg_[3 + a] + mc.sCoef * s[a];
    }
    bool smallOn = ADAM && !gateWord;
    if constexpr (SPARSE) smallOn = smallOn && myVis;
    if (smallOn) {
        float sp[14] = {m[0], m[1], m[2], sr[0], sr[1], sr[2], rr[0], rr[1], rr[2], rr[3], opr, d0v[0], d0v[1], d0v[2]};
        const float slr[14] = {adam.lr[0], adam.lr[0], adam.lr[0], adam.lr[3], adam.lr[3], adam.lr[3], adam.lr[4],
                               adam.lr[4], adam.lr[4], adam.lr[4], adam.lr[5], adam.lr[1], adam.lr[1], adam.lr[1]};
#pragma unroll
        for (int i = 0; i < 14; i++) adam_step(adam, sg_[i], slr[i], sp[i], sm_[i], sv_[i]);
        if constexpr (MCMC) {
            float dn[3];
            mcmc_noise(mc, (uint32_t)p, sp + 3, sp + 6, sp[10], dn);
            sp[0] = sp[0] + dn[0]; sp[1] = sp[1] + dn[1]; sp[2] = sp[2] + dn[2];
        }
        float* pB = const_cast<float*>(adam.pBase);
        auto out3 = [&](int i0) {
            const size_t o = small_off(i0);
            *reinterpret_cast<V3*>(pB + o) = V3{sp[i0], sp[i0 + 1], sp[i0 + 2]};
            *reinterpret_cast<V3*>(adam.mBase + o) = V3{sm_[i0], sm_[i0 + 1], sm_[i0 + 2]};
            *reinterpret_cast<V3*>(adam.vBase + o) = V3{sv_[i0], sv_[i0 + 1], sv_[i0 + 2]};
        };
        out3(0); out3(3); out3(11);
        {
            const size_t o = small_off(6);
            *reinterpret_cast<V4*>(pB + o) = V4{sp[6], sp[7], sp[8], sp[9]};
            *reinterpret_cast<V4*>(adam.mBase + o) = V4{sm_[6], sm_[7], sm_[8], sm_[9]};
            *reinterpret_cast<V4*>(adam.vBase + o) = V4{sv_[6], sv_[7], sv_[8], sv_[9]};
        }
        { const size_t o = small_off(10); pB[o] = sp[10]; adam.mBase[o] = sm_[10]; adam.vBase[o] = sv_[10]; }
    }
    }
    if (MODE == 0 && rows > 0 && L > 0) sh_rows_out(myRows, gFrest + (size_t)row0 * L, rows, L, lane);
    if (ADAM && !gateWord && rows > 0 && L > 0) {
        if (kept) adam_rows_kept<SPARSE>(adam, frest, row0, total4, L, myRows, lane, adam.lr[2], keptRows, visBits);
        else adam_rows<SPARSE>(adam, frest, row0, rows, L, myRows, lane, adam.lr[2], visBits);
    }
    if constexpr (POSE) {
        float* out = posePartials + 16 * ((size_t)blockIdx.x * (PROJ_FUSED_THREADS / 64) + wv);
#pragma unroll
        for (int j = 0; j < 15; j++) {
            const float t = wave_sum_xor(pose[j]);
            if (lane == j) out[j] = t;
        }
        if (lane == 15) out[15] = 0.f;
    }
}

constexpr bool proj_bwd_form_exists(int MODE, bool POSE, bool MCMC, bool F3D, bool SPARSE, bool FISHEYE = false)
{
    return (MODE == 0 || MODE == 1 || MODE == 2) &&
           (!FISHEYE || (!POSE && !F3D && MODE != 1)) &&
           (!POSE || MODE != 1) &&
           (!MCMC || MODE == 2) &&
           (!SPARSE || (MODE == 2 && !MCMC && !F3D)) &&
           (!F3D || (!MCMC && MODE != 1));
}

struct ProjBwdArgs {
    int N, K, degree;
    CamParams cam;
    const float *xyz, *fdc, *frest, *scalesRaw, *rotRaw, *opacityRaw, *gradAcc16;
    float *gXyz, *gFdc, *gFrest, *gScales, *gRot, *gOpacity;
    float* gradNormAccum;
    AdamFuse adam;
    float* posePartials;
    McmcFuse mc;
    const float* filter3d;
    const unsigned char* visMask;
    const CamParams* dcam;
};

template <int MODE, bool POSE, bool AA, bool MCMC, bool F3D, bool SPARSE, bool FISHEYE = false>
__global__ __launch_bounds__(PROJ_FUSED_THREADS) void proj_bwd_fused_kernel(ProjBwdArgs a)
{
    static_assert(proj_bwd_form_exists(MODE, POSE, MCMC, F3D, SPARSE, FISHEYE), "no such form of the fused projection backward");
    CamParams posed;
    if constexpr (POSE) posed = *a.dcam;
    proj_bwd_fused_body<MODE, POSE, AA, MCMC, F3D, SPARSE, FISHEYE>(a.N, a.K, a.degree, POSE ? posed : a.cam, a.xyz, a.fdc, a.frest, a.scalesRaw,
                                                           a.rotRaw, a.opacityRaw, a.gradAcc16, a.gXyz, a.gFdc, a.gFrest, a.gScales,
                                                           a.gRot, a.gOpacity, a.gradNormAccum, a.adam, a.posePartials, a.mc, a.filter3d,
                                                           a.visMask);
}

__global__ __launch_bounds__(256) void vis_mask_kernel(int N, const float* __restrict__ radii, unsigned char* __restrict__ mask)
{
    const int p = blockIdx.x * 256 + threadIdx.x;
    if (p < N) mask[p] = radii[p] > 0.0f ? 1 : 0;
}

__global__ __launch_bounds__(256) void color_cot_kernel(int N, const float* __restrict__ gradAcc16,
                                                        const float* __restrict__ packed12, float* __restrict__ out,
                                                        const uint32_t* __restrict__ ovf, float* __restrict__ rider)
{
    const int p = blockIdx.x * 256 + threadIdx.x;
    if (p == 0 && rider) *rider = *ovf ? 1.0f : 0.0f;
    if (p >= N) return;
    const float* ga = gradAcc16 + (size_t)p * 16;
    const uint32_t gate = __float_as_uint(packed12[(size_t)p * 12 + 11]);
    float4 r0 = *reinterpret_cast<const float4*>(ga), r1 = *reinterpret_cast<const float4*>(ga + 4), r2 = *reinterpret_cast<const float4*>(ga + 8);
    drop_nonfinite_row(r0, r1, r2);
    const float col[3] = {r1.z, r1.w, r2.x};
#pragma unroll
    for (int ch = 0; ch < 3; ch++) {
        const uint32_t side = (gate >> (2 * ch)) & 3u;
        const float g = col[ch];
        out[(size_t)p * 3 + ch] = side == 2u ? g : (side == 1u ? 0.5f * g : 0.0f);
    }
}

struct ViewCenters {
    float c[16][3];
    int n;
};

template <bool ADAM>
__global__ __launch_bounds__(PROJ_FUSED_THREADS) void sh_grad_from_views_kernel(
    int N, int K, int degree, ViewCenters views, const float* __restrict__ xyz, const float* __restrict__ mgAll,
    long long mgStride, float* gFdc, float* gFrest, const float* fdcParam, const float* frestParam, AdamFuse adam)
{
    extern __shared__ float shLds[];
    const uint32_t gateWord = (ADAM || adam.gwWords) ? adam_gate_word(adam) : 0u;
    adam_gate_publish(adam, gateWord);
    const int p = blockIdx.x * PROJ_FUSED_THREADS + threadIdx.x;
    const int lane = threadIdx.x & 63, wv = threadIdx.x >> 6;
    const int L = (K - 1) * 3;
    float* rest = shLds + wv * 64 * (L + 1) + lane * (L + 1);
    const int row0 = blockIdx.x * PROJ_FUSED_THREADS + wv * 64;
    const int rows = min(64, N - row0);
    if (p < N) {
        for (int i = 0; i < L; i++) rest[i] = 0.0f;
        float dc[3] = {0.f, 0.f, 0.f};
        const float m0 = xyz[3 * p], m1 = xyz[3 * p + 1], m2 = xyz[3 * p + 2];
        for (int r = 0; r < views.n; r++) {
            const float* mg = mgAll + (size_t)r * (size_t)mgStride + (size_t)p * 3;
// ... 278 lines not shown
    const bool colour = !c->rider.on && !selfColour;
    const size_t dynLds = c->rider.on ? 0 : colour ? lds : sizeof(float) * (PROJ_FUSED_THREADS / 64) * 64 * GS_RIDER_ROW;
    const int rc = with_flags(
        [&](auto TWO_PHASE, auto COLOUR, auto SELF, auto AA, auto F3D, auto POSE, auto FISHEYE) {
            if constexpr (proj_fwd_form_exists(TWO_PHASE, COLOUR, SELF, POSE, F3D, FISHEYE)) {
                hipLaunchKernelGGL((proj_fwd_fused_kernel<TWO_PHASE, COLOUR, SELF, AA, F3D, POSE, FISHEYE>), dim3(gs_div_up(N, PROJ_FUSED_THREADS)),
                                   dim3(PROJ_FUSED_THREADS), dynLds, c->stream, N, K, c->degree, cam, c->tileW, c->tileH,
                                   c->gridW, c->gridH, xyz, fdc, frest, scales, rot, opacity, c->packed12, radii, c->tileRect,
                                   c->tilesTouched, c->depthKey[0], c->depthVal[0], c->visPerBlock, c->counters, pflags, a, c->virt, cc,
                                   pieces, c->filter3d, c->poseCam);
                return GS_OK;
            } else {
                c->err = "fused projection forward: no kernel for this combination of settings";
                return GS_ERR_INVALID_ARG;
            }
        },
        !colour || twoPhase, colour, selfColour, c->antialias, c->filter3d != nullptr, posed, c->fisheye);
    if (rc) return rc;
    c->visBlocks = gs_div_up(N, PROJ_FUSED_THREADS);
    GS_HIP_CHECK(c, hipGetLastError());
    if (c->sparseAdam) return launch_vis_mask(c, N, radii);
    return GS_OK;
}

int launch_vis_mask(gs_ctx* c, int N, const float* radii)
{
    if (N == 0) return GS_OK;
    if (!radii || !c->visMask || N > c->visCap) { c->err = "sparse Adam: no visibility buffers for this forward"; return GS_ERR_INVALID_ARG; }
    hipLaunchKernelGGL(vis_mask_kernel, dim3(gs_div_up(N, 256)), dim3(256), 0, c->stream, N, radii, c->visMask);
    GS_HIP_CHECK(c, hipGetLastError());
    return GS_OK;
}

__global__ __launch_bounds__(GS_RIDER_WAVES * 64) void colour_rest_kernel(ColourRider r)
{
    colour_rider_block(r, (int)blockIdx.x);
}

int launch_colour_rest(gs_ctx* c)
{
    if (!c->rider.on) return GS_OK;
    c->rider.on = false;
    const int left = c->rider.total - c->rider.next;
    if (left <= 0) return GS_OK;
    ColourRider a = c->rider.args;
    a.unit0 = c->rider.next; a.units = left;
    c->rider.next = c->rider.total;
    hipLaunchKernelGGL(colour_rest_kernel, dim3(rider_blocks(left, GS_RIDER_WAVES * 64)), dim3(GS_RIDER_WAVES * 64), 0, c->stream, a);
    GS_HIP_CHECK(c, hipGetLastError());
    return GS_OK;
}

struct ProjBwdGrads { float *xyz, *fdc, *frest, *scales, *rot, *opacity; };
static int launch_proj_bwd_fused(gs_ctx* c, int mode, const ProjBwdGrads& g, const AdamFuse& adam)
{
    const int N = c->fwd.N, K = c->fwd.K;
    if (N == 0) return c->fwd.poseDelta && mode != 1 ? launch_pose_grad(c, 0) : GS_OK;
    const bool f3d = c->fwd.filter3d != nullptr;
    if (f3d && mode == 1) mode = 0;
    const bool pose = c->fwd.poseDelta && mode != 1;
    const bool mcmc = mode == 2 && !f3d && c->mcmcOn;
    const bool sparse = mode == 2 && !f3d && !mcmc && c->sparseAdam;
    ProjBwdArgs a = {};
    a.N = N; a.K = K; a.degree = c->degree;
    a.cam = c->fwd.cam; a.dcam = c->poseCam;
    a.xyz = c->fwd.xyz; a.fdc = c->fwd.fdc; a.frest = c->fwd.frest; a.scalesRaw = c->fwd.scales; a.rotRaw = c->fwd.rot;
    a.opacityRaw = c->fwd.opacity; a.gradAcc16 = c->gradAcc16;
    a.gXyz = g.xyz; a.gFdc = g.fdc; a.gFrest = g.frest; a.gScales = g.scales; a.gRot = g.rot; a.gOpacity = g.opacity;
    a.gradNormAccum = c->gradNormAccum;
    a.adam = adam;
    a.posePartials = c->posePartials;
    if (mcmc) a.mc = mcmc_fuse(c->mcmc, N, adam.lr[0]);
    a.filter3d = c->fwd.filter3d;
    a.visMask = c->visMask;
    const size_t lds = sizeof(float) * (PROJ_FUSED_THREADS / 64) * 64 * ((K - 1) * 3 + 1);
    const int rc = with_flags(
        [&](auto ADAM, auto EMIT_MG, auto POSE, auto AA, auto MCMC, auto F3D, auto SPARSE, auto FISHEYE) {
            constexpr int MODE = ADAM ? 2 : EMIT_MG ? 1 : 0;
            if constexpr (!(ADAM && EMIT_MG) && proj_bwd_form_exists(MODE, POSE, MCMC, F3D, SPARSE, FISHEYE)) {
                hipLaunchKernelGGL((proj_bwd_fused_kernel<MODE, POSE, AA, MCMC, F3D, SPARSE, FISHEYE>), dim3(gs_div_up(N, PROJ_FUSED_THREADS)),
                                   dim3(PROJ_FUSED_THREADS), lds, c->stream, a);
                return GS_OK;
            } else {
                c->err = "fused projection backward: no kernel for this combination of settings";
                return GS_ERR_INVALID_ARG;
            }
        },
        mode == 2, mode == 1, pose, c->fwd.antialias, mcmc, f3d, sparse, c->fwd.fisheye);
    if (rc) return rc;
    GS_HIP_CHECK(c, hipGetLastError());
    return pose ? launch_pose_grad(c, N) : GS_OK;
}

int launch_projection_fused_backward(gs_ctx* c, float* gXyz, float* gFdc, float* gFrest, float* gScales, float* gRot, float* gOpacity,
                                     bool emitColorCot)
{
    AdamFuse none = {};
    if (!emitColorCot) { none.ovf = c->counters + GS_CNT_OVERFLOW; none.rider = c->overflowRider; }
    return launch_proj_bwd_fused(c, emitColorCot ? 1 : 0, ProjBwdGrads{gXyz, gFdc, gFrest, gScales, gRot, gOpacity}, none);
}

int launch_projection_fused_backward_adam(gs_ctx* c, const float* pBase, float* mBase, float* vBase, const float lr[6], float b1,
                                          float b2, float eps, float gscale)
{
    AdamFuse a = {};
    a.pBase = pBase; a.mBase = mBase; a.vBase = vBase;
    for (int i = 0; i < 6; i++) a.lr[i] = lr[i];
    a.b1 = b1; a.b2 = b2; a.eps = eps; a.gscale = gscale;
    a.gate = c->adamGate;
    return launch_proj_bwd_fused(c, 2, ProjBwdGrads{}, a);
}

static long long cc_block_floats(const gs_ctx* c, int N) { return c->ccBlockFloats > 0 ? c->ccBlockFloats : 3LL * N; }
static void fill_gathered_gate(const gs_ctx* c, int N, const float* mgAll, AdamFuse& a)
{
    a.seen = c->gateSeen;
    if (c->ccBlockFloats <= 0) return;
    a.gwWords = reinterpret_cast<const uint32_t*>(mgAll + 3LL * N);
    a.gwStride = c->ccBlockFloats; a.gwCount = c->ccBlockCount; a.gwOut = c->gatheredGateOut;
}

int launch_color_cot(gs_ctx* c, int N, float* out)
{
    if (N == 0) return GS_OK;
    hipLaunchKernelGGL(color_cot_kernel, dim3(gs_div_up(N, 256)), dim3(256), 0, c->stream, N, c->gradAcc16, c->packed12,
                       out, c->counters + GS_CNT_OVERFLOW, c->overflowRider);
    GS_HIP_CHECK(c, hipGetLastError());
    return GS_OK;
}

int launch_sh_grad_from_views(gs_ctx* c, int N, int K, int R, const float* xyz, const float* mgAll,
                              const float* camCentersHost, float* gFdc, float* gFrest)
{
    if (N == 0) return GS_OK;
    ViewCenters v;
    v.n = R;
    for (int r = 0; r < R; r++) for (int k = 0; k < 3; k++) v.c[r][k] = camCentersHost[r * 3 + k];
    const size_t lds = sizeof(float) * (PROJ_FUSED_THREADS / 64) * 64 * ((K - 1) * 3 + 1);
    AdamFuse none = {};
    fill_gathered_gate(c, N, mgAll, none);
    hipLaunchKernelGGL(sh_grad_from_views_kernel<false>, dim3(gs_div_up(N, PROJ_FUSED_THREADS)), dim3(PROJ_FUSED_THREADS),
                       lds, c->stream, N, K, c->degree, v, xyz, mgAll, cc_block_floats(c, N), gFdc, gFrest, nullptr, nullptr, none);
    GS_HIP_CHECK(c, hipGetLastError());
    return GS_OK;
}

int launch_sh_grad_from_views_adam(gs_ctx* c, int N, int K, int R, const float* xyz, const float* mgAll,
                                   const float* camCentersHost, const float* fdcParam, const float* frestParam,
                                   const float* pBase, float* mBase, float* vBase, float lrDc, float lrRest, float b1,
                                   float b2, float eps, float gscale)
{
    if (N == 0) return GS_OK;
    ViewCenters v;
    v.n = R;
    for (int r = 0; r < R; r++) for (int k = 0; k < 3; k++) v.c[r][k] = camCentersHost[r * 3 + k];
    const size_t lds = sizeof(float) * (PROJ_FUSED_THREADS / 64) * 64 * ((K - 1) * 3 + 1);
    AdamFuse a = {};
    a.pBase = pBase; a.mBase = mBase; a.vBase = vBase;
    a.lr[1] = lrDc; a.lr[2] = lrRest;
    a.b1 = b1; a.b2 = b2; a.eps = eps; a.gscale = gscale;
    a.gate = c->adamGate;
    fill_gathered_gate(c, N, mgAll, a);
    hipLaunchKernelGGL(sh_grad_from_views_kernel<true>, dim3(gs_div_up(N, PROJ_FUSED_THREADS)), dim3(PROJ_FUSED_THREADS),
// ... 224 lines not shown
```

### gaussiansplattingmlx_amd/renderer.py

```python
from __future__ import annotations

import ctypes as C
import math
import os
from collections import OrderedDict, namedtuple

import numpy as np
import torch

from . import _lib, loss_mask
from ._lib import GsplatError

TILE_SIZE_H_W = namedtuple("TILE_SIZE_H_W", ["w", "h"])
RenderResult = namedtuple("RenderResult", ["render", "depth", "alpha", "visiility_filter", "radii"])


def _p(t):
    return None if t is None else C.c_void_p(t.data_ptr())


def _f32(t, device):
    if isinstance(t, torch.Tensor):
        return t.to(device=device, dtype=torch.float32).contiguous()
    return torch.as_tensor(np.ascontiguousarray(t, dtype=np.float32), device=device)


class CutPolicy:

    def __init__(self, min_dropped: int = 6_000_000, probe_interval: int = 64):
        self.min_dropped, self.probe_interval = min_dropped, probe_interval
        self.sit_out = 0
        self.last_dropped = 0
        self.since_empty = 0

    def begin(self, allowed: bool) -> bool:
        use = allowed and self.sit_out == 0 and self.since_empty >= 1
        if allowed and self.sit_out > 0:
            self.sit_out -= 1
        return use

    def renewed(self):
        self.since_empty += 1

    def report(self, missed: bool, kept: int, full: int):
        self.last_dropped = max(int(full) - int(kept), 0)
        if not missed and full > 0 and self.last_dropped < self.min_dropped:
            self.sit_out = self.probe_interval

    def cuts_cleared(self):
        self.since_empty = 0


class GaussianRenderer:
    def __init__(self, active_sh_degree: int, W: int, H: int, TILE_SIZE=TILE_SIZE_H_W(16, 16),
                 whiteBackground: bool = False, useScreenSpaceCustomOp: bool = True, device: int = 0,
                 antialiased: bool = False):
        self.lib = _lib.load()
        if not torch.cuda.is_available():
            raise RuntimeError("GaussianRenderer needs a GPU: the HIP path has no CPU fallback")
        self.active_sh_degree, self.W, self.H = int(active_sh_degree), int(W), int(H)
        self.TILE_SIZE = TILE_SIZE_H_W(*TILE_SIZE)
        self.whiteBackground = bool(whiteBackground)
        self.useScreenSpaceCustomOp = useScreenSpaceCustomOp
        self.device = torch.device("cuda", device)
        self.profiler = None
        torch.cuda.set_device(self.device)
        ctx = C.c_void_p()
        rc = self.lib.gs_ctx_create(device, self.W, self.H, self.TILE_SIZE.w, self.TILE_SIZE.h,
                                    self.active_sh_degree, int(self.whiteBackground), C.byref(ctx))
        if rc != _lib.GS_OK:
            raise GsplatError(rc, "gs_ctx_create failed")
        self.ctx = ctx
        self._check(self.lib.gs_ctx_set_stream(self.ctx, C.c_void_p(torch.cuda.current_stream(self.device).cuda_stream)))
        win = np.zeros(121, np.float32)
        self.lib.gs_ssim_window(11, C.c_float(1.5), win.ctypes.data_as(C.c_void_p))
        self.ssimWindow = torch.as_tensor(win, device=self.device)
        self._saved = {}
        self.reserved = None
        self._grad_norm_accum = None
        self._work_hints = {}
        self.depthCuts = True
        self._cut_policy = {}
        self._cut_view = None
        self._hinted_view = None
        self.cutMinDropped = 6_000_000
        self.cutProbeInterval = 64
        self._hints_ok = (self.TILE_SIZE.w, self.TILE_SIZE.h) == (16, 16) or \
            ((self.TILE_SIZE.w % 16 != 0 or self.TILE_SIZE.h % 16 != 0) and os.environ.get("GSPLAT_BLOCK_LISTS", "1") != "0")
        self.targetStatsCache = True
        self._target_cache = OrderedDict()
        self.targetStatsCacheBytes = 8 << 30
        self._antialiased = False
        self._camera_model = "pinhole"
        self._absgrad = False
        self._sparse_adam = False
        self._background = None
        self._exposure = (None, None)
        self._bilateral = (None, None)
        self._loss_mask = None
        if antialiased:
            self.setAntialiased(True)

    def close(self):
        if getattr(self, "ctx", None):
            self.lib.gs_set_block_work_buffer(self.ctx, None)
            self.lib.gs_set_loss_target_cache(self.ctx, None, 0)
            self.lib.gs_set_loss_mask(self.ctx, None)
            self.lib.gs_set_grad_norm_accum(self.ctx, None)
            self.lib.gs_ctx_destroy(self.ctx)
            self.ctx = None

    def __del__(self):
        try:
            self.close()
        except Exception:
            pass

    def _check(self, rc):
        if rc != _lib.GS_OK:
            raise GsplatError(rc, self.lib.gs_last_error(self.ctx).decode())

    def _t(self, t):
        return _f32(t, self.device)

    def _measure(self, name, body):
        return self.profiler.measure(name, body) if self.profiler is not None else body()

    def _empty(self, *shape, dtype=torch.float32):
        return torch.empty(shape, dtype=dtype, device=self.device)

    def reserve(self, max_gaussians: int, max_pairs: int):
        self._check(self.lib.gs_ctx_reserve(self.ctx, int(max_gaussians), int(max_pairs)))
        self.reserved = (int(max_gaussians), int(max_pairs))

    def sync(self):
        self._check(self.lib.gs_sync(self.ctx))

    _TUNING = dict(fwd_waves_per_simd=_lib.TUNE_FWD_WAVES_PER_SIMD, bwd_waves_per_cu=_lib.TUNE_BWD_WAVES_PER_CU,
                   fwd_quadrants=_lib.TUNE_FWD_QUADRANTS, op_fwd_ppl=_lib.TUNE_OP_FWD_PPL,
                   op_bwd_ppl=_lib.TUNE_OP_BWD_PPL, fwd_trace_buffer=_lib.TUNE_FWD_TRACE_BUFFER,
                   depth_gradient=_lib.TUNE_DEPTH_GRADIENT, wide_tile_sort=_lib.TUNE_WIDE_TILE_SORT,
                   host_overflow_errors=_lib.TUNE_HOST_OVERFLOW_ERRORS, splitter_depth_sort=_lib.TUNE_SPLITTER_DEPTH_SORT,
                   colour_riders=_lib.TUNE_COLOUR_RIDERS, fwd_queues=_lib.TUNE_FWD_QUEUES, fwd_four_waves=_lib.TUNE_FWD_FOUR_WAVES,
                   fwd_fold_test_scale=_lib.TUNE_FWD_FOLD_TEST_SCALE, poison_checkpoints=_lib.TUNE_POISON_CHECKPOINTS,
                   render_only=_lib.TUNE_RENDER_ONLY, fwd_pair=_lib.TUNE_FWD_PAIR, fwd_slow_slot=_lib.TUNE_FWD_SLOW_SLOT,
                   trim_rects=_lib.TUNE_TRIM_RECTS)
    _TUNING_DEFAULTS = dict(fwd_waves_per_simd=4, bwd_waves_per_cu=16, fwd_quadrants=1, op_fwd_ppl=1, op_bwd_ppl=1,
                            fwd_trace_buffer=0, depth_gradient=1, wide_tile_sort=1, host_overflow_errors=1, splitter_depth_sort=1,
                            colour_riders=1, fwd_queues=8, fwd_four_waves=-1, fwd_fold_test_scale=1000, poison_checkpoints=0, render_only=0, fwd_pair=-1, fwd_slow_slot=3, trim_rects=2)

    def setTuning(self, **knobs):
        for k, v in knobs.items():
            self._check(self.lib.gs_ctx_set_tuning(self.ctx, self._TUNING[k], int(v)))
            self._tuning_now = {**getattr(self, "_tuning_now", {}), k: int(v)}

    def getTuning(self, knob: str) -> int:
        return getattr(self, "_tuning_now", {}).get(knob, self._TUNING_DEFAULTS[knob])

    def colourRidersActive(self, N: int, K: int = 25) -> bool:
        if K != 25 or self.getTuning("colour_riders") != 1 or ((self.TILE_SIZE.w % 16 or self.TILE_SIZE.h % 16) and not self.blockLists):
            return False
        return bool(self.getTuning("splitter_depth_sort")) and 16384 < N <= 160 * 4096

    def stats(self):
        s = (C.c_uint32 * 8)()
        self._check(self.lib.gs_last_stats(self.ctx, s))
        return dict(N_visible=s[0], M=s[1], max_tile_list=s[2], overflow=s[5], capN=s[6], capM=s[7])

    @staticmethod
    def _camera(viewMatrix, projMatrix, cameraCenter, fovX, fovY, focalX, focalY):
        g = lambda a: a.detach().cpu().numpy() if isinstance(a, torch.Tensor) else a
        return _lib.make_camera(g(viewMatrix), g(projMatrix), g(cameraCenter), float(g(fovX)), float(g(fovY)),
                                float(g(focalX)), float(g(focalY)))

    def get_scales_from(self, scales):
        return torch.exp(scales)

    def get_rotation_from(self, rotation):
        return rotation / (torch.sqrt(torch.sum(rotation * rotation, dim=1, keepdim=True)) + 1e-8)

    def get_xyz_from(self, xyz):
        return xyz

    def get_features_from(self, features_dc, features_rest):
        return torch.cat([features_dc, features_rest], dim=1)

    def get_opacity_from(self, opacity):
        return torch.sigmoid(opacity)

    def projectionScreenFused(self, scales, rotations, means3d, shs, cam):
        scales, rotations, means3d, shs = map(self._t, (scales, rotations, means3d, shs))
        N, K = means3d.shape[0], shs.shape[1]
        out = dict(means2d=self._empty(N, 2), depths=self._empty(N), color=self._empty(N, 3),
                   cov2d=self._empty(N, 2, 2), conic=self._empty(N, 2, 2), radii=self._empty(N),
                   rectMin=self._empty(N, 2), rectMax=self._empty(N, 2))
        self._check(self.lib.gs_projection_forward(
            self.ctx, N, K, _p(scales), _p(rotations), _p(means3d), _p(shs), C.byref(cam), _p(out["means2d"]),
            _p(out["depths"]), _p(out["color"]), _p(out["cov2d"]), _p(out["conic"]), _p(out["radii"]),
            _p(out["rectMin"]), _p(out["rectMax"])))
        return out

    def projectionScreenFusedVJP(self, scales, rotations, means3d, shs, cam, cotMeans2d, cotDepths, cotColor,
# ... 95 lines not shown
        maxW, sumW = self._empty(N).zero_(), self._empty(N).zero_()
        for i, cam in enumerate(cameras):
            self.renderChecked(params, cam, viewKey=None if viewKeys is None else viewKeys[i], wantDepth=False)
            self.renderContrib(maxW, sumW)
        return maxW, sumW

    def contribActions(self, score, threshold: float):
        score = self._t(score)
        N = int(score.shape[0])
        actions, counts = self._empty(N, dtype=torch.int32), self._empty(N, dtype=torch.int32)
        self._check(self.lib.gs_contrib_actions(self.ctx, N, _p(score), C.c_float(threshold), _p(actions), _p(counts)))
        return actions, counts

    def render(self, imageWidth, imageHeight, means2d, cov2d, color, opacity, depths, radii, conic, rect,
               inputIsDepthSorted: bool = False):
        if imageWidth != self.W or imageHeight != self.H:
            raise GsplatError(2, f"Renderer image size mismatch: expected ({self.W}, {self.H}), got "
                                 f"({imageWidth}, {imageHeight})")
        packed = self.buildPackedGaussians(means2d, conic, color, opacity, depths)
        radii_t, depths_t = self._t(radii), self._t(depths)
        N = radii_t.shape[0]
        self._check(self.lib.gs_tile_bin(self.ctx, N, _p(self._t(rect[0])), _p(self._t(rect[1])), _p(radii_t),
                                         _p(depths_t)))
        c, d, a = self.globalTileComposite(packed)
        return RenderResult(c.view(self.H, self.W, 3), d.view(self.H, self.W, 1), a.view(self.H, self.W, 1),
                            radii_t > 0, radii_t)

    def forwardWithCameraParams(self, viewMatrix, projMatrix, cameraCenter, fovX, fovY, focalX, focalY, imageWidth,
                                imageHeight, means3d, shs, opacity, scales, rotations):
        cam = self._camera(viewMatrix, projMatrix, cameraCenter, fovX, fovY, focalX, focalY)
        scales, rotations, means3d, shs = map(self._t, (scales, rotations, means3d, shs))
        o = self.projectionScreenFused(scales, rotations, means3d, shs, cam)
        res = self.render(imageWidth, imageHeight, o["means2d"], o["cov2d"], o["color"], opacity, o["depths"],
                          o["radii"], o["conic"], (o["rectMin"], o["rectMax"]))
        self._chain = dict(cam=cam, scales=scales, rotations=rotations, means3d=means3d, shs=shs, blend=self._saved)
        return res

    def forwardWithCameraParamsVJP(self, cotRender, cotDepth=None, cotAlpha=None):
        ch = self._chain
        gp = self.globalTileCompositeVJP(cotRender, cotDepth, cotAlpha, saved=ch["blend"])
        N = gp.shape[0]
        pb = self.projectionScreenFusedVJP(ch["scales"], ch["rotations"], ch["means3d"], ch["shs"], ch["cam"],
                                           gp[:, 0:2], gp[:, 10], gp[:, 6:9], torch.zeros(N, 4, device=self.device),
                                           gp[:, 2:6])
        return dict(means3d=pb["gradMeans3d"], shs=pb["gradShs"], opacity=gp[:, 9].contiguous(), scales=pb["gradScales"],
                    rotations=pb["gradRot"], gradPacked=gp, gradCameraCenter=pb["gradCameraCenter"])

    def forward(self, camera, means3d, shs, opacity, scales, rotations):
        return self.forwardWithCameraParams(camera.worldViewTransform, camera.projectionMatrix, camera.cameraCenter,
                                            camera.FoVx, camera.FoVy, camera.focalX, camera.focalY,
                                            camera.imageWidth, camera.imageHeight, means3d, shs, opacity, scales,
                                            rotations)

    def renderForward(self, params: dict, camera, want_radii: bool = False, viewKey=None, depthCuts: bool = True,
                      wantDepth: bool = True):
        cam = camera if isinstance(camera, _lib.gs_camera) else self._camera(
            camera.worldViewTransform, camera.projectionMatrix, camera.cameraCenter, camera.FoVx, camera.FoVy,
            camera.focalX, camera.focalY)
        model = getattr(camera, "model", "pinhole")
        if model != self._camera_model:
            self.setCameraModel(model)
        p = {k: (v if isinstance(v, torch.Tensor) and v.is_cuda and v.dtype == torch.float32 and v.is_contiguous()
                 else self._t(v)) for k, v in params.items()}
        N = p["xyz"].shape[0]
        K = 1 + p["features_rest"].shape[1]
        P = self.W * self.H
        if getattr(self, "_fbuf", None) is None:
            self._fbuf = (self._empty(P, 3), self._empty(P), self._empty(P))
        color, depth, alpha = self._fbuf
        radii = self._empty(N) if want_radii else None
        buf = None
        if viewKey is not None and self._hints_ok:
            buf = self._work_hints.get(viewKey)
            if buf is None:
                n = C.c_int()
                self._check(self.lib.gs_view_hint_words(self.ctx, C.byref(n)))
                buf = self._work_hints[viewKey] = torch.zeros(n.value, dtype=torch.int32, device=self.device)
        self._check(self.lib.gs_set_view_hints(self.ctx, _p(buf), 0 if buf is None else int(buf.numel())))
        use = False
        if buf is not None:
            pol = self._cut_policy.get(viewKey)
            if pol is None:
                pol = self._cut_policy[viewKey] = CutPolicy(self.cutMinDropped, self.cutProbeInterval)
            pol.min_dropped, pol.probe_interval = self.cutMinDropped, self.cutProbeInterval
            use = pol.begin(depthCuts and self.depthCuts)
        self._cut_view = viewKey if use else None
        self._hinted_view = viewKey if buf is not None else None
        self._check(self.lib.gs_set_depth_cuts(self.ctx, 1 if use else 0))
        self._check(self.lib.gs_render_forward(self.ctx, N, K, _p(p["xyz"]), _p(p["features_dc"]),
                                               _p(p["features_rest"]), _p(p["scales"]), _p(p["rotation"]),
                                               _p(p["opacity"]), C.byref(cam), _p(color),
                                               _p(depth if wantDepth else None), _p(alpha), _p(radii)))
        self._fused = dict(params=p, color=color, depth=depth if wantDepth else None, alpha=alpha, radii=radii)
        return RenderResult(color.view(self.H, self.W, 3), depth.view(self.H, self.W, 1) if wantDepth else None,
                            alpha.view(self.H, self.W, 1), None if radii is None else radii > 0, radii)

    def dropDepthCuts(self):
        for pol in self._cut_policy.values():
            pol.cuts_cleared()

    def _cuts_renewed(self):
        if self._hinted_view is not None:
            pol = self._cut_policy.get(self._hinted_view)
            if pol is not None:
                pol.renewed()

    def forwardMissed(self) -> bool:
        if os.environ.get("GSPLAT_DEBUG_NO_MISS_CHECK"):
            return False
        m = C.c_int()
        self._check(self.lib.gs_forward_missed(self.ctx, C.byref(m)))
        if self._cut_view is not None:
            st = (C.c_uint32 * 2)()
            self._check(self.lib.gs_cut_stats(self.ctx, st))
            self._cut_policy[self._cut_view].report(bool(m.value), int(st[0]), int(st[1]))
            self._cut_view = None
        return bool(m.value)

    def renderChecked(self, params: dict, camera, want_radii: bool = False, viewKey=None, wantDepth: bool = True):
        res = self.renderForward(params, camera, want_radii, viewKey, wantDepth=wantDepth)
        if self.forwardMissed():
            res = self.renderForward(params, camera, want_radii, viewKey, depthCuts=False, wantDepth=wantDepth)
        return res

    @property
    def blockLists(self) -> bool:
        return (self.TILE_SIZE.w % 16 != 0 or self.TILE_SIZE.h % 16 != 0) and os.environ.get("GSPLAT_BLOCK_LISTS", "1") != "0"

    def blockWork(self):
        n = C.c_int()
        self._check(self.lib.gs_block_count(self.ctx, C.byref(n)))
        out = self._empty(n.value, dtype=torch.int32)
        self._check(self.lib.gs_copy_block_work(self.ctx, _p(out)))
        return out

    def lastContrib(self):
        out = self._empty(self.H, self.W, dtype=torch.int32)
        self._check(self.lib.gs_copy_last_contrib(self.ctx, _p(out)))
        return out

    STAGES = ("proj_fwd", "bin", "blend_fwd", "loss", "blend_bwd", "proj_bwd", "adam")
# ... 680 lines not shown
```

### gaussiansplattingmlx_amd/trainer.py

```python
from __future__ import annotations

import ctypes as C
import math

import numpy as np
import torch

from ._lib import GS_ERR_REPLICA_MISMATCH, GsplatError
from .renderer import GaussianRenderer, _p

GS_ERR_WORKSPACE_OVERFLOW = 3

PARAM_ORDER = ("xyz", "features_dc", "features_rest", "scales", "rotation", "opacity")
ARENA_ORDER = ("xyz", "scales", "rotation", "opacity", "features_dc", "features_rest")


def getLearningRates(current: int, total: int):
    return [0.00016 * max(1.0 - float(current) / float(total), 0.01), 0.0025, 0.0025 / 20, 0.005, 0.001, 0.025]


def arenaLearningRates(current: int, total: int):
    lr = dict(zip(PARAM_ORDER, getLearningRates(current, total)))
    return [lr[k] for k in ARENA_ORDER]


def exposureLearningRate(current: int, total: int, lr=(0.01, 0.001)) -> float:
    s = min(float(current) / float(total), 1.0) if total > 0 else 1.0
    return math.exp((1.0 - s) * math.log(lr[0]) + s * math.log(lr[1]))


def bilateralGridLearningRate(current: int, total: int, lr: float = 2e-3) -> float:
    s = min(float(current) / float(total), 1.0) if total > 0 else 1.0
    return lr * (0.01 + 0.99 * min(current, 1000) / 1000.0) * 0.01 ** s


def view_for(step: int, rank: int, world: int, n_views: int) -> int:
    return (step * world + rank) % n_views


def balanced_view_order(costs):
    order = sorted(range(len(costs)), key=lambda v: (costs[v], v))
    return order[0::2] + order[1::2][::-1]


def cc_block_floats(N: int) -> int:
    return (3 * int(N) + 1 + 3) & ~3


def exchange_sh_compressed(grad_geom: torch.Tensor, cc_local: torch.Tensor, cc_all: torch.Tensor, process_group=None):
    import torch.distributed as dist
    dist.all_gather_into_tensor(cc_all.view(-1), cc_local.view(-1), group=process_group)
    dist.all_reduce(grad_geom, op=dist.ReduceOp.SUM, group=process_group)


def gathered_gate(cc_all: torch.Tensor, N: int) -> bool:
    return bool((cc_all.view(cc_all.shape[0], -1)[:, 3 * int(N)] != 0).any().item())


def allreduce_gradients(grad_arena: torch.Tensor, process_group=None) -> float:
    import torch.distributed as dist
    world = dist.get_world_size(process_group)
# ... 52 lines not shown
    both = torch.cat([w, -w])
    work = dist.all_reduce(both, op=dist.ReduceOp.MAX, group=process_group, async_op=True)
    return (w, both, work)


def check_replicas_end(pending, process_group=None, rank: int | None = None):
    import torch.distributed as dist
    w, both, work = pending
    work.wait()
    mine = [float(x) for x in w.cpu()]
    hi, lo = [float(x) for x in both[:3].cpu()], [-float(x) for x in both[3:].cpu()]
    if hi == lo:
        return
    _raise_replica_mismatch(hi, lo, mine, dist.get_rank(process_group) if rank is None else rank)


def _raise_replica_mismatch(hi, lo, mine, rank):
    names = ("N", "sum", "magnitudes")
    diff = " ".join(n for n, h, l in zip(names, hi, lo) if h != l)
    raise ReplicaMismatch(f"the ranks hold different models ({diff}): over the ranks N in [{lo[0]:.0f}, {hi[0]:.0f}], sum in "
                          f"[{lo[1]!r}, {hi[1]!r}], sum of magnitudes in [{lo[2]!r}, {hi[2]!r}]; rank {rank} has N = {mine[0]:.0f}, "
                          f"sum = {mine[1]!r}, sum of magnitudes = {mine[2]!r}")


def exchange_summary(dp_impl, dp_exchange, world, N, geom_numel, numel, steps, sums, counts, rccl_version, source, views_per_rank=1):
    n = max(int(steps), 1)
    per = lambda k: round(sums[k] / counts[k], 4) if counts.get(k) else None
    xg, xr = sums["exposed_gather"] / n, sums["exposed_reduce"] / n
    out = dict(dp_impl=dp_impl, dp_exchange=dp_exchange, world=int(world), steps_measured=int(steps), rccl_version=rccl_version,
               timing_source=source, gate_ms=per("gate"), gather_ms=per("gather"), reduce_ms=per("reduce"),
               exposed_gather_ms=round(xg, 4), exposed_reduce_ms=round(xr, 4), exposed_ms=round(xg + xr, 4))
    if dp_exchange == "sh_compressed":
        blk = 4 * cc_block_floats(N) * int(views_per_rank)
        out.update(gather_bytes_out=blk, gather_bytes_in=blk * int(world), reduce_bytes=4 * int(geom_numel),
                   collectives_per_step=2, gate_rides_in="gather", views_per_rank=int(views_per_rank))
    else:
        out.update(gather_bytes_out=0, gather_bytes_in=0, reduce_bytes=4 * (int(numel) + 1), collectives_per_step=1,
                   gate_rides_in="reduce")
    out["gate_bytes"] = 4
    return out


class GaussModel:

    def __init__(self, params: dict, device, capacity: int | None = None):
        self.device = device
        self._row = {k: tuple(params[k].shape[1:]) for k in ARENA_ORDER}
        self._per = {k: int(np.prod(self._row[k])) if len(self._row[k]) else 1 for k in ARENA_ORDER}
        self.floats_per_gaussian = int(sum(self._per.values()))
        self.K = self._row["features_rest"][0] + 1
        N = int(params["xyz"].shape[0])
        self._pbuf = [None, None]
        self._cur = 0
        self._gbuf = self._mbuf = self._vbuf = None
        self._mspare = self._vspare = None
        self._staged = None
        self.stride = N
        self._layout(N, max(int(capacity or N), N))
        for k in ARENA_ORDER:
            src = params[k]
            if not isinstance(src, torch.Tensor):
                src = torch.as_tensor(np.ascontiguousarray(src, np.float32))
            self._views[k].copy_(src.reshape(self._views[k].shape))

    def _buf(self, old, floats, zero=False):
        if old is not None and old.numel() >= floats + 4:
            return old
        return (torch.zeros if zero else torch.empty)(max(floats, 4) + 4, dtype=torch.float32, device=self.device)

    def _offsets(self, N: int):
        starts, off = [], 0
        for k in ARENA_ORDER:
            starts.append(off)
            off += (N * self._per[k] + 3) & ~3
        return starts, off

    def _zero_pads(self, buf, N):
        starts, total = self._offsets(N)
        for k, off, nxt in zip(ARENA_ORDER, starts, starts[1:] + [total]):
            if off + N * self._per[k] < nxt:
                buf[off + N * self._per[k]:nxt].zero_()

    def _carve(self, buf, N, stride=None):
        views = {}
        starts, _ = self._offsets(N if stride is None else stride)
        for k, off in zip(ARENA_ORDER, starts):
            n = N * self._per[k]
            views[k] = buf[off:off + n].view((N,) + self._row[k])
        return views

    def _layout(self, N: int, capacity: int, pads=("arena", "grad", "m", "v"), stride=None):
        stride = N if stride is None else int(stride)
        floats = self._offsets(max(capacity, stride))[1]
        self.capacity = capacity
        self.N = N
        self.stride = stride
        starts, self.numel = self._offsets(stride)
        self.seg_start = np.asarray(starts, np.int64)
        self.seg_end = np.asarray(starts[1:] + [self.numel], np.int64)
        self.geom_numel = int(self.seg_end[3])
        self._pbuf[self._cur] = self._buf(self._pbuf[self._cur], floats, zero=True)
        self._gbuf, self._mbuf, self._vbuf = (self._buf(b, floats, zero=True) for b in (self._gbuf, self._mbuf, self._vbuf))
        self.arena = self._pbuf[self._cur][:self.numel]
        self.grad, self.m, self.v = self._gbuf[:self.numel], self._mbuf[:self.numel], self._vbuf[:self.numel]
        if stride == N:
            for name in pads:
                self._zero_pads(getattr(self, name), N)
        self._views, self._gviews = self._carve(self.arena, N, stride), self._carve(self.grad, N, stride)

    def getParams(self):
        return self._views

    def getGrads(self):
        return self._gviews

    def stagingViews(self, N_new: int, stride=None) -> dict:
        cap = self.capacity if N_new <= self.capacity else int(N_new * 1.5)
        stride = N_new if stride is None else int(stride)
        other = 1 - self._cur
        self._pbuf[other] = self._buf(self._pbuf[other], self._offsets(max(cap, stride))[1], zero=True)
        self._staged = (N_new, cap, stride)
        return self._carve(self._pbuf[other][:self._offsets(stride)[1]], N_new, stride)

    def stagingBase(self, capacity: int):
        cap = max(int(capacity), self.capacity)
        other = 1 - self._cur
        self._pbuf[other] = self._buf(self._pbuf[other], self._offsets(cap)[1], zero=True)
        self._staged = (None, cap, None)
        return self._pbuf[other]

    def getMoments(self):
        return self._carve(self.m, self.N, self.stride), self._carve(self.v, self.N, self.stride)

    def stagingMoments(self):
        N_new, cap, stride = self._staged
        if N_new is None or stride != N_new:
            raise ValueError("stagingMoments: after stagingViews(N_new) in the packed layout")
        floats = self._offsets(max(cap, stride))[1]
        self._mspare, self._vspare = self._buf(self._mspare, floats, zero=True), self._buf(self._vspare, floats, zero=True)
        n = self._offsets(stride)[1]
        return self._carve(self._mspare[:n], N_new, stride), self._carve(self._vspare[:n], N_new, stride)

    def commitStaged(self, N_new=None, zero=True, moments=False):
        n_staged, cap, stride = self._staged
        N_new = n_staged if N_new is None else int(N_new)
        self._staged = None
# ... 244 lines not shown
        self.exchange_impl = exchange_impl
        self.model, self.gaussRender = model, gaussRender
        self.dp_exchange = dp_exchange
        self.iterationCount = iterationCount
        self.lambda_dssim = lambda_dssim
        self.pg = process_group
        self.world = 1
        self.rank = 0
        if process_group is not None:
            import torch.distributed as dist
            self.world = dist.get_world_size(process_group)
            self.rank = dist.get_rank(process_group)
        if dp_bootstrap is not None:
            _, self.rank, self.world = dp_bootstrap
        r = gaussRender
        self._loss = r._empty(4)
        self._cot = r._empty(r.H, r.W, 3)
        self._cotDepth = self._cotAlpha = None
        if self.depth is not None:
            self._cotDepth = r._empty(r.H, r.W)
            if self.depth.mode != "accumulated":
                self._cotAlpha = r._empty(r.H, r.W)
        self._seg_end = (C.c_longlong * 6)(*[int(x) for x in model.seg_end])
        self.iteration = 0
        self.gradientThreshold, self.minOpacity, self.maxScale = 0.0002, 0.005, 0.01
        if self.adc is not None:
            self.gradientThreshold, self.minOpacity = float(self.adc.grad_threshold), float(self.adc.min_opacity)
        if self.absgrad is not None:
            self.gradientThreshold = float(self.absgrad.threshold)
        self.densifyFromIter, self.densifyUntilIter, self.maxGaussians = 500, 15000, 1_000_000
        self.split_and_prune_per_iteration = 100
        self.densify = densify
        self.fuse_adam = fuse_adam
        self.outputDirectory = None
        self.save_snapshot_per_iteration = 100
        self.noise_seed = 20260313
        import os
        self.plannedDensify = os.environ.get("GSPLAT_PLANNED_DENSIFY", "1") != "0"
        self.noiseSource = None
        self.xyzGradAccumulation = r._empty(model.N).zero_()
        self.denomGradAccumulation = 0
        self.lastDensifyStats = None
        self.forwardMisses = 0
        self.enableIntervalProfiling = False
        self.profilingLogInterval = 100
        self.profilingTopKSections = 12
        self.lastProfileReport = None
        self.log = None
        self._committed = False
        self._referenceParamReload = False
        self._committed_params = None
        self.overflowRecoveries = 0
        self._checked_views = set()
        self._exchange = (process_group is not None or dp_bootstrap is not None) and (self.world > 1 or exchange_when_single)
        self._native = self._exchange and exchange_impl == "native"
        self._dp = self._exchange or self.viewsPerRank > 1
        self.inlineGather = False
        if self._exchange and not self._native and process_group is not None:
            import torch.distributed as dist
            self.inlineGather = (dist.get_backend(process_group) == "nccl" and
                                 os.environ.get("GSPLAT_DP_INLINE_GATHER", "1") != "0")
        if self._native:
            self._dp_connect(dp_bootstrap)
        if self._dp and dp_exchange == "sh_compressed":
            if self.world * self.viewsPerRank > 16:
                raise ValueError("sh_compressed exchange supports at most 16 views per step (ranks x views_per_rank)")
        self._gate = None
        self.overflowCheckInterval = 16
        self._xt = None
        if self._dp and not self._native:
            self._gate = torch.zeros(1, dtype=torch.int32, device=r.device)
            self._seen = torch.zeros(1, dtype=torch.int32, device=r.device)
            self._need = torch.zeros(1, dtype=torch.int64, device=r.device)
        self._alloc_exchange_buffers()
        if self.mcmc is not None:
            model.restride(max(self.mcmc.cap_max, model.capacity))
            self._seg_end = (C.c_longlong * 6)(*[int(x) for x in model.seg_end])
        self._perView = {}
        eye = torch.eye(3, 4, dtype=torch.float32).reshape(12)
        if self.pose_opt:
            self.nViews, self.poseLr = int(n_views), (float(pose_lr[0]), float(pose_lr[1]))
            self._perView["pose_opt"] = _PerViewTable("pose_opt", n_views, 6, r.device, (3, 6), lambda it, total: self.poseLr,
                                                      GaussianRenderer.setPoseCorrection)
            self._pose_delta = self._perView["pose_opt"].rows
        if self.exposure_opt:
            self.nViews, self.exposureLr = int(n_views), elr
            self._perView["exposure_opt"] = _PerViewTable(
                "exposure_opt", n_views, 12, r.device, (12,), lambda it, total: (exposureLearningRate(it, total, self.exposureLr),),
                GaussianRenderer.setExposure, start=eye)
            self._expo_m, self._expo_v = self._perView["exposure_opt"].m, self._perView["exposure_opt"].v
        if self.bilateral_grid:
            self.nViews, self.bilateralGridShape = int(n_views), bgs
            self.bilateralGridLr, self.bilateralGridTv = blr, btv
            nodes = bgs[0] * bgs[1] * bgs[2]
            self._perView["bilateral_grid"] = _PerViewTable(
                "bilateral_grid", n_views, nodes * 12, r.device, (nodes * 12,),
                lambda it, total: (bilateralGridLearningRate(it, total, self.bilateralGridLr),),
                lambda rr, G, g: rr.setBilateralGrid(G, g, self.bilateralGridShape, self.bilateralGridTv),
                start=eye.repeat(nodes), shared_grad=True)
            self._bg_m, self._bg_v = self._perView["bilateral_grid"].m, self._perView["bilateral_grid"].v
        self._filter = None
        if self.filter_3d:
            self.filter3dInterval = int(filter_3d_interval)
            r.setFilterCameras(list(filter_cameras))
            self._updateFilter3D()
        if self._exchange:
# ... 616 lines not shown
        st = dict(ev={}, work={})
        self._xt.append(st)
        return st

    @staticmethod
    def _xt_mark(st, name):
        if st is not None:
            e = torch.cuda.Event(enable_timing=True)
            e.record()
            st["ev"][name] = e

    def exchangeTimingRead(self):
        if self._xt is None:
            return None
        r, m = self.gaussRender, self.model
        if self._native:
            ms, steps, ver = (C.c_float * 8)(), C.c_int(), C.c_int()
            r._check(r.lib.gs_dp_exchange_read(r.ctx, ms, C.byref(steps), C.byref(ver)))
            r._check(r.lib.gs_dp_exchange_timing(r.ctx, 0))
            sums = dict(gate=ms[0], gather=ms[1], reduce=ms[2], exposed_gather=ms[3], exposed_reduce=ms[4])
            counts = dict(gate=steps.value, gather=steps.value, reduce=steps.value)
            n, version = steps.value, ver.value
            source = ("HIP events on the library's side stream around each RCCL call, and on the ctx stream around its "
                      "hipStreamWaitEvent on them (gs_dp_exchange_read)")
        else:
            torch.cuda.synchronize(r.device)
            n = len(self._xt)
            sums = dict(gate=0.0, gather=0.0, reduce=0.0, exposed_gather=0.0, exposed_reduce=0.0)
            counts = dict(gate=0, gather=0, reduce=0)
            for st in self._xt:
                ev = st["ev"]
                for a, b, k in (("wg0", "wg1", "exposed_gather"), ("wr0", "wr1", "exposed_reduce")):
                    if a in ev and b in ev:
                        sums[k] += ev[a].elapsed_time(ev[b])
                for k, w in st["work"].items():
                    try:
                        sums[k] += float(w._get_duration())
                        counts[k] += 1
                    except Exception:
                        pass
            try:
                import torch.cuda.nccl as _nccl
                v = _nccl.version()
                version = v[0] * 10000 + v[1] * 100 + v[2] if isinstance(v, tuple) else int(v)
            except Exception:
                version = None
            source = ("torch.cuda events on the render stream around every Work.wait(); collective durations from "
                      "Work._get_duration() (null where the backend keeps none)")
        self._xt = None
        return exchange_summary(self.exchange_impl, self.dp_exchange, self.world, m.N, int(m.geom_numel), int(m.numel), n, sums,
                                counts, version, source, self.viewsPerRank)

    def trainStep(self, camera, targetRGB, stepCameras=None, viewKey=None, targetAlpha=None, lossMask=None, targetDepth=None,
                  depthMask=None, depthAlign=(1.0, 0.0)):
        if getattr(camera, "model", "pinhole") == "fisheye":
            for on, name in ((self.pose_opt, "pose_opt"), (self.filter_3d, "filter_3d")):
                if on:
                    raise ValueError(f"trainStep: a fisheye camera does not go with {name} (pinhole cameras only)")
            if self.pg is not None or self.exchange_impl == "native":
                raise ValueError("trainStep: a fisheye camera takes single-device steps only (no process group, dp_bootstrap or "
                                 "native exchange)")
            if self.viewsPerRank != 1:
                raise ValueError("trainStep: a fisheye camera takes one view per step only (views_per_rank > 1 is not supported)")
        if lossMask is not None:
            if self.viewsPerRank != 1:
                raise ValueError("trainStep: lossMask takes one view per step only (views_per_rank > 1 is not supported)")
            if self.pg is not None or self.exchange_impl == "native":
                raise ValueError("trainStep: lossMask takes single-device steps only (no process group, dp_bootstrap or native exchange)")
        if (targetAlpha is None) != (self.background is None):
            raise ValueError("trainStep: targetAlpha goes with a trainer built with background=BackgroundConfig(...)"
                             if self.background is None else
                             "trainStep: a trainer built with background= needs targetAlpha (the view's alpha, [H, W])")
        depth = self.depth
        if (targetDepth is None) != (depth is None):
            raise ValueError("trainStep: targetDepth goes with a trainer built with depth=DepthConfig(...)"
                             if depth is None else
                             "trainStep: a trainer built with depth= needs targetDepth (the view's depth map, [H, W])")
        if depth is None and depthMask is not None:
            raise ValueError("trainStep: depthMask goes with a trainer built with depth=DepthConfig(...)")
        profiled = self.enableIntervalProfiling and (self.iteration % self.profilingLogInterval == 0
                                                     or self.iteration == self.iterationCount - 1)
        step = self._profiledStep if profiled else (self._trainStepMulti if self.viewsPerRank > 1 else self._trainStep)
        r = self.gaussRender
        restore = dict(depth_gradient=r.getTuning("depth_gradient"), host_overflow_errors=r.getTuning("host_overflow_errors"))
        sparse_was = getattr(r, "_sparse_adam", False)
        bg_was = mask_was = None
        if self.background is not None:
            b = self.background.color_at(self.iteration)
            bg_was = (getattr(r, "_background", None),)
            targetRGB = self._compositeTarget(targetRGB, targetAlpha, b)
        tables = list(self._perView.values())
        row = tables[0].row(viewKey) if tables else None
        try:
            if depth is not None:
                self._depthStep = self._depthInputs(targetDepth, depthMask, depthAlign)
            r.setTuning(depth_gradient=0 if depth is None else 1)
            if self.mcmc is not None:
                r.setMCMC(self._mcmcParams())
            if self.filter_3d:
                r.setFilter3D(self._filter)
            if self.sparse_adam and not sparse_was:
                r.setSparseAdam(True)
            if self.background is not None:
                r.setBackground(b)
                self.lastBackground = b
            for t in tables:
                t.bindRow(r, row)
# ... 118 lines not shown
            body = self._trainStepMulti if self.viewsPerRank > 1 else self._trainStep
            out = prof.measure("train.valueAndGrad.execute", lambda: body(camera, targetRGB, stepCameras, viewKey))
            prof.setDeviceStages(r.profileRead())
        finally:
            r.profile(False)
            r.profiler = None
        self.lastProfileReport = prof.makeReport(it, time.perf_counter_ns() - t0, self.profilingTopKSections, 0.01)
        self.lastProfiler = prof
        if self.log:
            self.log(self.lastProfileReport)
        return out

    def _nativeStep(self, stepCameras):
        from . import _lib
        r, m = self.gaussRender, self.model
        a = _lib.gs_dp_step_args()
        a.cot_color, a.cot_depth, a.cot_alpha = self._cot.data_ptr(), None, None
        a.params_base, a.grads_base, a.m_base, a.v_base = (t.data_ptr() for t in (m.arena, m.grad, m.m, m.v))
        a.n_arena, a.geom_numel, a.nseg = int(m.numel), int(m.geom_numel), 6
        for i, (e, lr) in enumerate(zip(m.seg_end, arenaLearningRates(self.iteration, self.iterationCount))):
            a.seg_end[i], a.seg_lr[i] = int(e), float(lr)
        a.beta1, a.beta2, a.eps = 0.9, 0.999, 1e-15
        mode = _lib.GS_DP_ALLREDUCE
        if self.dp_exchange == "sh_compressed":
            if stepCameras is None or len(stepCameras) != self.world:
                raise ValueError("sh_compressed exchange needs stepCameras (one camera per rank, rank order)")
            centres = np.ascontiguousarray(np.stack([np.asarray(getattr(c, "cameraCenter", c), np.float32).reshape(3)
                                                     for c in stepCameras]), np.float32)
            a.cam_centers = centres.ctypes.data
            a.color_cot_local, a.color_cot_all = self._cc_local.data_ptr(), self._cc_all.data_ptr()
            mode = _lib.GS_DP_SH_COMPRESSED
        r._cuts_renewed()
        r._check(r.lib.gs_dp_step(r.ctx, mode, C.byref(a)))

    def _beginIteration(self):
        r, m = self.gaussRender, self.model
        if self.referenceParamReload and self._committed_params is None:
            self._committed_params = m.arena.clone()
        if self.densify:
            if self.xyzGradAccumulation.shape[0] != m.N:
                self.resetGradientAccumulation()
            if getattr(r, "_grad_norm_accum", None) is not self.xyzGradAccumulation:
                r.setGradNormAccum(self.xyzGradAccumulation)
        elif getattr(r, "_grad_norm_accum", None) is not None:
            r.setGradNormAccum(None)
        if self.absgrad is not None and not getattr(r, "_absgrad", False):
            r.setAbsgrad(True)
        if self.adc is not None and self.iteration <= self.adc.densify_until:
            r.setADCStats(*self._adcAccumulators())

    def _forwardAndLoss(self, camera, targetRGB, viewKey, lossOut):
        r, m = self.gaussRender, self.model
        wd = self._depthStep is not None
        res = r._measure("train.forward", lambda: r.renderForward(m.getParams(), camera, viewKey=viewKey, wantDepth=wd))
        if viewKey is not None and viewKey not in self._checked_views:
            self._checked_views.add(viewKey)
            if self.checkOverflow():
                res = r.renderForward(m.getParams(), camera, viewKey=viewKey, wantDepth=wd)
        r._measure("train.loss.total", lambda: r.lossForwardBackward(res.render, targetRGB, self.lambda_dssim,
                                                                      out=dict(loss=lossOut, cotColor=self._cot),
                                                                      targetKey=self._lossTargetKey(viewKey)))
        if wd:
            self._depthLoss(res, lossOut)
        if viewKey is not None and r.forwardMissed():
            self.forwardMisses += 1
            res = r.renderForward(m.getParams(), camera, viewKey=viewKey, depthCuts=False, wantDepth=wd)
            r.lossForwardBackward(res.render, targetRGB, self.lambda_dssim, out=dict(loss=lossOut, cotColor=self._cot),
                                  targetKey=self._lossTargetKey(viewKey))
            if wd:
                self._depthLoss(res, lossOut)

    def _geometryAdam(self, lr: dict, scale: float):
        r, m = self.gaussRender, self.model
        glr = (C.c_float * 4)(lr["xyz"], lr["scales"], lr["rotation"], lr["opacity"])
        r._check(r.lib.gs_adam_step_add(r.ctx, m.geom_numel, _p(m.arena), _p(m.grad), _p(m.m), _p(m.v), 4,
                                        (C.c_longlong * 4)(*[int(x) for x in m.seg_end[:4]]), glr, C.c_float(0.9), C.c_float(0.999),
                                        C.c_float(1e-15), C.c_float(scale), _p(self._xyz_add), 3 * m.N))

    def _trainStepMulti(self, cameras, targets, stepCameras=None, viewKeys=None):
        r, m = self.gaussRender, self.model
        V, N = self.viewsPerRank, m.N
        if len(cameras) != V or len(targets) != V or (viewKeys is not None and len(viewKeys) != V):
            raise ValueError(f"views_per_rank = {V}: trainStep takes {V} cameras, targets and view keys")
        total = self.world * V
        if stepCameras is None and not self._exchange:
            stepCameras = cameras
        if stepCameras is None or len(stepCameras) != total:
            raise ValueError(f"sh_compressed exchange needs stepCameras: {total} cameras (ranks x views_per_rank, rank-major)")
        self._beginIteration()
        ccf = cc_block_floats(N)
        blocks = self._cc_local.view(V, ccf)
        for j in range(V):
            key = None if viewKeys is None else viewKeys[j]
            self._forwardAndLoss(cameras[j], targets[j], key, self._loss_v[j])
            r._check(r.lib.gs_set_overflow_rider(r.ctx, C.c_void_p(blocks[j].data_ptr() + 12 * N)))
            if self.fuse_adam:
                r.renderBackwardDPGeom(self._cot, blocks[j], self._geom_views[j], self._xyz_own[j])
            else:
                r.renderBackwardDPBegin(self._cot, colorCot=blocks[j])
                r.renderBackwardDPFinish(out=self._geom_views[j])
            if self.densify:
                self.addGradientAccumulation()
        g_geom = m.grad[:m.geom_numel]
        torch.sum(self._geom_v, dim=0, out=g_geom)
        reduce = None
        xt = self._xt_step() if self._exchange else None
        if self._exchange:
            import torch.distributed as dist
            gather = self._gatherColourCotangents(xt)
            reduce = dist.all_reduce(g_geom, op=dist.ReduceOp.SUM, group=self.pg, async_op=True)
            if xt is not None:
                xt["work"].update(reduce=reduce)
            self._awaitGather(gather, xt)
        centres = np.stack([np.asarray(getattr(c, "cameraCenter", c), np.float32).reshape(3) for c in stepCameras])
        scale = 1.0 / total
        if self.fuse_adam:
            lr = dict(zip(PARAM_ORDER, getLearningRates(self.iteration, self.iterationCount)))
            own = [None] * total
            for j in range(V):
                own[self.rank * V + j] = self._xyz_own[j]
            r.shGradFromViewsAdamDir(m.getParams(), self._cc_all, centres, own, m.arena, m.m, m.v, lr["features_dc"],
                                     lr["features_rest"], scale, self._xyz_add)
            if reduce is not None:
                self._xt_mark(xt, "wr0")
                reduce.wait()
                self._xt_mark(xt, "wr1")
            self._geometryAdam(lr, scale)
        else:
            r.shGradFromViews(m.getParams()["xyz"], self._cc_all, centres, m.K, out=m.getGrads())
            if reduce is not None:
                reduce.wait()
            lrs = (C.c_float * 6)(*arenaLearningRates(self.iteration, self.iterationCount))
            r._check(r.lib.gs_adam_step(r.ctx, m.numel, _p(m.arena), _p(m.grad), _p(m.m), _p(m.v), 6, self._seg_end, lrs,
                                        C.c_float(0.9), C.c_float(0.999), C.c_float(1e-15), C.c_float(scale)))
        torch.mean(self._loss_v, dim=0, out=self._loss)
        return self._finishIteration()

    def _depthCots(self) -> dict:
        if self._depthStep is None:
            return {}
        return dict(cotDepth=self._cotDepth, cotAlpha=self._cotAlpha)

    def _trainStep(self, camera, targetRGB, stepCameras=None, viewKey=None):
        r, m = self.gaussRender, self.model
        self._beginIteration()
        self._forwardAndLoss(camera, targetRGB, viewKey, self._loss)
        xt = None
        if self._gate is not None:
            xt = self._xt_step()
        fused = False
        if self._native:
            self._nativeStep(stepCameras)
            if self.densify:
                self.addGradientAccumulation()
            fused = True
        elif not self._exchange and self.fuse_adam:
            r._measure("bwd.fused+train.optimizer.applySingle", lambda: r.renderBackwardAdam(
                self._cot, m.arena, m.m, m.v, getLearningRates(self.iteration, self.iterationCount), **self._depthCots()))
            if self.densify:
                self.addGradientAccumulation()
            fused = True
        elif not self._exchange:
            r.renderBackward(self._cot, out=m.getGrads(), **self._depthCots())
            if self.mcmc is not None:
                g = m.getGrads()
                r.mcmcRegularizerGrad(m.getParams()["scales"], m.getParams()["opacity"], g["scales"], g["opacity"],
                                      self._mcmcParams())
            if self.densify:
                self.addGradientAccumulation()
        elif self.dp_exchange == "allreduce":
            r.renderBackward(self._cot, out=m.getGrads())
            if self.densify:
                self.addGradientAccumulation()
            self._xt_mark(xt, "wr0")
            allreduce_gradients(m._gbuf[:m.numel + 1], self.pg)
            self._xt_mark(xt, "wr1")
        else:
            if stepCameras is None or len(stepCameras) != self.world:
                raise ValueError("sh_compressed exchange needs stepCameras (one camera per rank, rank order)")
            import torch.distributed as dist
            g = m.getGrads()
            if self.fuse_adam:
                r.renderBackwardDPGeom(self._cot, self._cc_local, g, self._xyz_own[0])
                gather = self._gatherColourCotangents(xt)
            else:
                r.renderBackwardDPBegin(self._cot, colorCot=self._cc_local)
                gather = self._gatherColourCotangents(xt, inline=False)
                r.renderBackwardDPFinish(out=g)
            if self.densify:
                self.addGradientAccumulation()
            reduce = dist.all_reduce(m.grad[:m.geom_numel], op=dist.ReduceOp.SUM, group=self.pg, async_op=True)
            centres = np.stack([np.asarray(getattr(c, "cameraCenter", c), np.float32).reshape(3) for c in stepCameras])
            if xt is not None:
                xt["work"].update(reduce=reduce)
            self._awaitGather(gather, xt)
            if self.fuse_adam:
                lr = dict(zip(PARAM_ORDER, getLearningRates(self.iteration, self.iterationCount)))
                own = [self._xyz_own[0] if q == self.rank else None for q in range(self.world)]
                r.shGradFromViewsAdamDir(m.getParams(), self._cc_all, centres, own, m.arena, m.m, m.v, lr["features_dc"],
                                         lr["features_rest"], 1.0 / self.world, self._xyz_add)
                self._xt_mark(xt, "wr0")
                reduce.wait()
                self._xt_mark(xt, "wr1")
                self._geometryAdam(lr, 1.0 / self.world)
                fused = True
            else:
                r.shGradFromViews(m.getParams()["xyz"], self._cc_all, centres, m.K, out=g)
                self._xt_mark(xt, "wr0")
                reduce.wait()
                self._xt_mark(xt, "wr1")
        if not fused and self.sparse_adam:
            lrs = (C.c_float * 6)(*arenaLearningRates(self.iteration, self.iterationCount))
            widths = (C.c_int * 6)(*[max(int(m._per[k]), 1) for k in ARENA_ORDER])
            r._check(r.lib.gs_adam_step_visible(r.ctx, m.numel, _p(m.arena), _p(m.grad), _p(m.m), _p(m.v), 6, self._seg_end, lrs,
                                                widths, C.c_float(0.9), C.c_float(0.999), C.c_float(1e-15), C.c_float(1.0),
                                                m.N, None))
        elif not fused:
            lrs = (C.c_float * 6)(*arenaLearningRates(self.iteration, self.iterationCount))
            r._check(r.lib.gs_adam_step(r.ctx, m.numel, _p(m.arena), _p(m.grad), _p(m.m), _p(m.v), 6, self._seg_end, lrs,
                                        C.c_float(0.9), C.c_float(0.999), C.c_float(1e-15), C.c_float(1.0 / self.world)))
            if self.mcmc is not None:
                p = m.getParams()
                r.mcmcInjectNoise(p["xyz"], p["scales"], p["rotation"], p["opacity"],
                                  getLearningRates(self.iteration, self.iterationCount)[0], self._mcmcParams())
        for t in self._perView.values():
            t.adam(r, int(viewKey), self.iteration, self.iterationCount)
        return self._finishIteration()

    def _finishIteration(self):
        r, m = self.gaussRender, self.model
        it = self.iteration
        self.iteration += 1
        if self.outputDirectory is not None and it % self.save_snapshot_per_iteration == 0:
            self.save_snapshot(it)
        if self.mcmc is not None and self.mcmc.is_event(it):
            self._mcmcEvent(it)
            if self._overflow_reported():
                self.checkOverflow()
        if self.adc is not None:
            if self.adc.is_event(it):
                self._adcEvent(it)
                if self._overflow_reported():
                    self.checkOverflow()
            if self.adc.is_reset(it):
                self._adcResetOpacity()
        moved = False
        if self.densify and it % self.split_and_prune_per_iteration == 0:
            self._committed = False
            self.split_and_prune(it)
            moved = self._committed
            if not self._committed:
                m.resetOptimizerState()
                if self.referenceParamReload and self._committed_params is not None \
                        and self._committed_params.numel() == m.arena.numel():
                    m.arena.copy_(self._committed_params)
                    moved = True
            if self._exchange and not self._plans_events():
                self._collectiveOverflowCheck(force=self._committed)
            elif self._exchange:
                pass
            elif self._overflow_reported():
                self.checkOverflow()
        if self.contribPrune is not None and self.contribPrune.is_event(it):
            self._contribPruneEvent(self.contribPrune.cameras, self.contribPrune.threshold, self.contribPrune.score)
            moved = moved or self._committed
        if self.filter_3d and (moved or self.iteration % self.filter3dInterval == 0):
            self._updateFilter3D()
        return self._loss
```

### include/gsplat.h

```cpp
#ifndef GSPLAT_H
#define GSPLAT_H

#include <stddef.h>
#include <stdint.h>

#ifdef __cplusplus
extern "C" {
#endif

#define GSPLAT_ABI_VERSION 6

typedef enum gs_status {
    GS_OK = 0,
    GS_ERR_INVALID_ARG = 1,
    GS_ERR_SIZE_MISMATCH = 2,
    GS_ERR_WORKSPACE_OVERFLOW = 3,
    GS_ERR_HIP = 4,
    GS_ERR_NO_FORWARD = 5,
    GS_ERR_NO_DEVICE = 6,
    GS_ERR_IO = 7,
    GS_ERR_COMM = 8,
    GS_ERR_REPLICA_MISMATCH = 9
} gs_status;

// ... 30 lines not shown
                           const float* cot_depths, const float* cot_means2d, const float* cot_cov2d,
                           const float* cot_color, const float* cot_conic, float* grad_scales,
                           float* grad_rotations, float* grad_means3d, float* grad_shs,
                           float* grad_cam_center_point);


int gs_tile_bin(gs_ctx* ctx, int N, const float* rect_min, const float* rect_max, const float* radii,
                const float* depths);
int gs_tile_bin_cut(gs_ctx* ctx, int N, const float* rect_min, const float* rect_max, const float* radii,
                    const float* depths, const uint32_t* tile_cuts);
int gs_tile_bin_info(gs_ctx* ctx, uint32_t* M , uint32_t* B );
int gs_tile_bin_views(gs_ctx* ctx, const uint32_t** sorted_gauss_idx, const uint32_t** tile_ranges,
                      const uint32_t** tile_counts);
int gs_tile_bin_export(gs_ctx* ctx, uint32_t* sorted_gauss_idx, uint32_t* tile_ranges, uint32_t* tile_counts);
int gs_build_packed_tile_indices(gs_ctx* ctx, uint32_t B, int32_t* out);


int gs_pack_gaussians(gs_ctx* ctx, int N, const float* means2d, const float* conic, const float* color,
                      const float* opacity, const float* depths, float* packed );

int gs_blend_forward(gs_ctx* ctx, int N, const float* packed , float* out_color, float* out_depth,
                     float* out_alpha, uint32_t* last_contrib);

int gs_blend_backward(gs_ctx* ctx, int N, const float* packed, const float* cot_color, const float* cot_depth,
                      const float* cot_alpha, const float* out_color, const float* out_depth,
                      const float* out_alpha, const uint32_t* last_contrib, float* grad_packed);

int gs_blend_contrib(gs_ctx* ctx, int N, const float* packed , float* max_w ,
                     float* sum_w );


int gs_ssim_window(int K, float sigma, float* window );
int gs_ssim_forward(gs_ctx* ctx, int H, int W, int C, int K, const float* img1, const float* img2,
                    const float* window , float* out_ssim, float* out_mu1, float* out_mu2,
                    float* out_sigma1, float* out_sigma2, float* out_sigma12);
int gs_ssim_backward(gs_ctx* ctx, int H, int W, int C, int K, const float* grad_out, const float* img1,
                     const float* img2, const float* window, const float* mu1, const float* mu2,
                     const float* sigma1, const float* sigma2, const float* sigma12, float* grad_img1,
                     float* grad_img2);


int gs_render_forward(gs_ctx* ctx, int N, int K, const float* xyz, const float* features_dc,
                      const float* features_rest, const float* scales, const float* rotation,
                      const float* opacity, const gs_camera* cam , float* out_color, float* out_depth,
                      float* out_alpha, float* radii);

int gs_render_backward(gs_ctx* ctx, const float* cot_color, const float* cot_depth, const float* cot_alpha,
                       float* grad_xyz, float* grad_features_dc, float* grad_features_rest, float* grad_scales,
                       float* grad_rotation, float* grad_opacity);

int gs_render_backward_adam(gs_ctx* ctx, const float* cot_color, const float* cot_depth, const float* cot_alpha,
                            float* params_base, float* m_base, float* v_base, long long n_arena, const float lr[6],
                            float beta1, float beta2, float eps, float grad_scale);

int gs_render_contrib(gs_ctx* ctx, float* max_w , float* sum_w );

int gs_set_pose_correction(gs_ctx* ctx, const float* delta , float* grad_delta );

int gs_set_exposure(gs_ctx* ctx, const float* M , float* grad );
int gs_apply_exposure(gs_ctx* ctx, long long n_pixels, const float* M , const float* in, float* out);

int gs_set_bilateral_grid(gs_ctx* ctx, const float* grid , float* grad , int grid_w,
                          int grid_h, int grid_l, float tv_weight);
int gs_apply_bilateral_grid(gs_ctx* ctx, int W, int H, const float* grid , int grid_w, int grid_h, int grid_l,
                            const float* in , float* out );

int gs_set_antialiasing(gs_ctx* ctx, int enable);

#define GS_CAMERA_PINHOLE 0
#define GS_CAMERA_FISHEYE 1
int gs_set_camera_model(gs_ctx* ctx, int model);
int gs_get_camera_model(gs_ctx* ctx, int* model );

int gs_set_background(gs_ctx* ctx, const float* rgb );
int gs_get_background(gs_ctx* ctx, float rgb[3] );
int gs_composite_target(gs_ctx* ctx, long long n_pixels, const float* rgb , const float* alpha ,
                        const float* bg , float* out );

int gs_set_absgrad(gs_ctx* ctx, int enable);
int gs_get_absgrad(gs_ctx* ctx, int N, float* out );

int gs_set_sparse_adam(gs_ctx* ctx, int enable);
int gs_get_visibility(gs_ctx* ctx, int N, unsigned char* out );

int gs_set_filter3d_cameras(gs_ctx* ctx, int V, const gs_camera* cams );
int gs_compute_filter3d(gs_ctx* ctx, int N, const float* xyz , float* filter );
int gs_set_filter3d(gs_ctx* ctx, const float* filter );
int gs_filter3d_bake(gs_ctx* ctx, int N, const float* scales_raw , const float* opacity_raw ,
                     const float* filter , float* out_scales_raw , float* out_opacity_raw );

typedef struct gs_lens { float fx, fy, cx, cy, k1, k2, p1, p2; float dst_fx, dst_fy, dst_cx, dst_cy; } gs_lens;
int gs_undistort(gs_ctx* ctx, const gs_lens* lens , int src_w, int src_h, int dst_w, int dst_h, int channels,
                 int mode, const void* src , void* dst , unsigned char* valid );

typedef struct gs_fisheye_lens { float fx, fy, cx, cy, k1, k2, k3, k4; float dst_fx, dst_fy, dst_cx, dst_cy; } gs_fisheye_lens;
int gs_undistort_fisheye(gs_ctx* ctx, const gs_fisheye_lens* lens , int src_w, int src_h, int dst_w, int dst_h, int channels,
                         int mode, const void* src , void* dst , unsigned char* valid );

typedef struct gs_mcmc_params {
    double noise_lr;
    double opacity_reg;
    double scale_reg;
    double min_opacity;
    double grow_rate;
    long long cap_max;
    int n_max;
// ... 184 lines not shown
int gs_ply_pack_rows(gs_ctx* ctx, int N, int K, const float* xyz, const float* features_dc,
                     const float* features_rest, const float* opacity, const float* scales, const float* rotation,
                     float* rows);

int gs_dist_topk(gs_ctx* ctx, int N, int k, int q_begin, int q_count, const float* xyz, float* out);


typedef enum gs_stage {
    GS_STAGE_PROJ_FWD = 0,
    GS_STAGE_BIN = 1,
    GS_STAGE_BLEND_FWD = 2,
    GS_STAGE_LOSS = 3,
    GS_STAGE_BLEND_BWD = 4,
    GS_STAGE_PROJ_BWD = 5,
    GS_STAGE_ADAM = 6,
    GS_STAGE_COUNT = 8
} gs_stage;
int gs_profile_enable(gs_ctx* ctx, unsigned stage_mask);
int gs_profile_read(gs_ctx* ctx, float ms[GS_STAGE_COUNT] , int calls[GS_STAGE_COUNT] );

int gs_last_stats(gs_ctx* ctx, uint32_t stats[8] );
int gs_set_block_work_buffer(gs_ctx* ctx, uint32_t* buf);
int gs_view_hint_words(gs_ctx* ctx, int* n);
int gs_set_view_hints(gs_ctx* ctx, uint32_t* buf, int words);
int gs_clear_depth_cuts(gs_ctx* ctx, uint32_t* buf, int words);
int gs_set_depth_cuts(gs_ctx* ctx, int enable);
int gs_forward_missed(gs_ctx* ctx, int* missed );
int gs_cut_stats(gs_ctx* ctx, uint32_t out[2] );
int gs_set_grad_norm_accum(gs_ctx* ctx, float* accum);
int gs_copy_overflow_flag(gs_ctx* ctx, uint32_t* out );
int gs_set_update_gate(gs_ctx* ctx, const uint32_t* gate );
int gs_set_overflow_rider(gs_ctx* ctx, float* dst );
int gs_set_gathered_gate(gs_ctx* ctx, long long block_floats, int count, uint32_t* reduced_out );
int gs_set_gate_seen(gs_ctx* ctx, uint32_t* seen );

typedef enum gs_tuning {
    GS_TUNE_FWD_WAVES_PER_SIMD = 0,
    GS_TUNE_BWD_WAVES_PER_CU = 1,
    GS_TUNE_FWD_QUADRANTS = 2,
    GS_TUNE_OP_FWD_PPL = 3,
    GS_TUNE_OP_BWD_PPL = 4,
    GS_TUNE_FWD_TRACE_BUFFER = 5,
    GS_TUNE_WIDE_TILE_SORT = 7,
    GS_TUNE_HOST_OVERFLOW_ERRORS = 8,
    GS_TUNE_SPLITTER_DEPTH_SORT = 9,
    GS_TUNE_COLOUR_RIDERS = 10,
    GS_TUNE_FWD_QUEUES = 11,
    GS_TUNE_FWD_FOUR_WAVES = 12,
    GS_TUNE_FWD_FOLD_TEST_SCALE = 13,
    GS_TUNE_RENDER_ONLY = 15,
    GS_TUNE_FWD_PAIR = 16,
    GS_TUNE_FWD_SLOW_SLOT = 17,
    GS_TUNE_TRIM_RECTS = 18,
    GS_TUNE_POISON_CHECKPOINTS = 14,
    GS_TUNE_DEPTH_GRADIENT = 6
} gs_tuning;
int gs_ctx_set_tuning(gs_ctx* ctx, int knob, long long value);

int gs_block_count(gs_ctx* ctx, int* n);
int gs_copy_block_work(gs_ctx* ctx, uint32_t* out);
int gs_copy_last_contrib(gs_ctx* ctx, uint32_t* out);

#ifdef __cplusplus
}
#endif
#endif
```

Measured before the change: 619.4.

## Project next training view inside fused backward+Adam kernel and adopt it in forward

While the fused projection backward+Adam kernel has the freshly updated parameters in registers, it also runs the next view's projection (geometry, tile rects, SH colour, depth keys) and writes the results to a spare workspace. The next forward pass checks that the parameters, camera and flags match and then swaps in those buffers instead of launching its own projection pass. This removes one full read of all Gaussian parameters and a kernel launch per step. In exchange the backward kernel carries more registers and work, extra device buffers are allocated, and the host must predict the next camera through a view-successor guess.

Measured after the change: 632.4 (median of 6 runs). 1.02x the previous value.

```diff
diff --git a/gaussiansplattingmlx_amd/_lib.py b/gaussiansplattingmlx_amd/_lib.py
--- a/gaussiansplattingmlx_amd/_lib.py
+++ b/gaussiansplattingmlx_amd/_lib.py
@@ -102,6 +102,9 @@
     "gs_render_backward": (C.c_int, [_vp] + [_vp] * 9),
     "gs_render_backward_dp": (C.c_int, [_vp] + [_vp] * 8),
     "gs_render_backward_adam": (C.c_int, [_vp] * 7 + [C.c_longlong, _vp, C.c_float, C.c_float, C.c_float, C.c_float]),
+    "gs_set_next_view": (C.c_int, [_vp, C.POINTER(gs_camera)]),
+    "gs_accept_next_view": (C.c_int, [_vp]),
+    "gs_next_view_stats": (C.c_int, [_vp, C.POINTER(C.c_uint32)]),
     "gs_render_backward_dp_begin": (C.c_int, [_vp] * 5),
     "gs_render_backward_dp_finish": (C.c_int, [_vp] * 5),
     "gs_render_backward_dp_finish_geom": (C.c_int, [_vp] * 6),
@@ -219,7 +222,7 @@
 
 TUNE_FWD_WAVES_PER_SIMD, TUNE_BWD_WAVES_PER_CU, TUNE_FWD_QUADRANTS, TUNE_OP_FWD_PPL, TUNE_OP_BWD_PPL, \
     TUNE_FWD_TRACE_BUFFER, TUNE_DEPTH_GRADIENT, TUNE_WIDE_TILE_SORT, TUNE_HOST_OVERFLOW_ERRORS, TUNE_SPLITTER_DEPTH_SORT, \
-    TUNE_COLOUR_RIDERS, TUNE_FWD_QUEUES, TUNE_FWD_FOUR_WAVES, TUNE_FWD_FOLD_TEST_SCALE, TUNE_POISON_CHECKPOINTS, TUNE_RENDER_ONLY, TUNE_FWD_PAIR, TUNE_FWD_SLOW_SLOT, TUNE_TRIM_RECTS = range(19)
+    TUNE_COLOUR_RIDERS, TUNE_FWD_QUEUES, TUNE_FWD_FOUR_WAVES, TUNE_FWD_FOLD_TEST_SCALE, TUNE_POISON_CHECKPOINTS, TUNE_RENDER_ONLY, TUNE_FWD_PAIR, TUNE_FWD_SLOW_SLOT, TUNE_TRIM_RECTS, TUNE_NEXT_VIEW = range(20)
 
 
 def exported_symbols():
diff --git a/gaussiansplattingmlx_amd/csrc/api.hip b/gaussiansplattingmlx_amd/csrc/api.hip
--- a/gaussiansplattingmlx_amd/csrc/api.hip
+++ b/gaussiansplattingmlx_amd/csrc/api.hip
@@ -4,6 +4,7 @@
 #include <string.h>
 
 #include "gs_ctx.h"
+#include <utility>
 #include <vector>
 
 using namespace gs;
@@ -31,6 +32,15 @@
 {
     if (p) (void)hipFree(p);
     p = nullptr;
+}
+
+void free_next_view_ws(gs_ctx* c)
+{
+    GsNextView& v = c->nextView;
+    dev_free(v.packed12); dev_free(v.tileRect); dev_free(v.tilePieces); dev_free(v.tilesTouched); dev_free(v.depthKey);
+    dev_free(v.depthVal); dev_free(v.visPerBlock);
+    v.cap = 0;
+    v.ready = false;
 }
 
 void free_gaussian_ws(gs_ctx* c)
@@ -42,6 +52,7 @@
     dev_free(c->bucketId);
     dev_free(c->densifyTiles);
     c->densifyTileCap = 0;
+    free_next_view_ws(c);
 }
 
 void free_pair_ws(gs_ctx* c)
@@ -404,6 +415,52 @@
 }
 
 #pragma GCC visibility push(default)
+static int ensure_next_view_ws(gs_ctx* c)
+{
+    GsNextView& v = c->nextView;
+    if (v.cap == c->capN && v.packed12) return GS_OK;
+    GS_HIP_CHECK(c, hipStreamSynchronize(c->stream));
+    free_next_view_ws(c);
+    const size_t n = (size_t)c->capN;
+    int rc;
+    if ((rc = dev_alloc(c, &v.packed12, n * 12))) return rc;
+    if ((rc = dev_alloc(c, &v.tileRect, n))) return rc;
+    if ((rc = dev_alloc(c, &v.tilePieces, n))) return rc;
+    if ((rc = dev_alloc(c, &v.tilesTouched, n))) return rc;
+    if ((rc = dev_alloc(c, &v.depthKey, n))) return rc;
+    if ((rc = dev_alloc(c, &v.depthVal, n))) return rc;
+    if ((rc = dev_alloc(c, &v.visPerBlock, n / 128 + 2))) return rc;
+    v.cap = c->capN;
+    return GS_OK;
+}
+
+static bool next_view_matches(const gs_ctx* c, int N, int K, const float* const ptr[6], const CamParams& cp, const float* radii)
+{
+    const GsNextView& v = c->nextView;
+    if (!v.enabled || !v.accept || !v.ready || v.cap != c->capN || N != v.N || K != v.K || radii) return false;
+    for (int i = 0; i < 6; i++) if (ptr[i] != v.ptr[i]) return false;
+    if (memcmp(&cp, &v.cam, sizeof(CamParams)) != 0) return false;
+    if (c->fwd.cutsActive || c->poseDelta || c->antialias || c->fisheye || c->filter3d || c->sparseAdam || c->adcGradSum || c->virt.nbx ||
+        !c->fast16)
+        return false;
+    bool pieces = false;
+    return next_view_flags(c, N, &pieces) == v.flags && pieces == v.pieces;
+}
+
+static int adopt_next_view(gs_ctx* c, int N)
+{
+    GsNextView& v = c->nextView;
+    std::swap(c->packed12, v.packed12); std::swap(c->tileRect, v.tileRect); std::swap(c->tilePieces, v.tilePieces);
+    std::swap(c->tilesTouched, v.tilesTouched); std::swap(c->depthKey[0], v.depthKey); std::swap(c->depthVal[0], v.depthVal);
+    std::swap(c->visPerBlock, v.visPerBlock);
+    c->rider.on = false;
+    c->dropBlocks = 0;
+    c->piecesValid = v.pieces;
+    c->visBlocks = gs_div_up(N, 128);
+    v.accepted++;
+    return zero_counters(c);
+}
+
 extern "C" {
 
 int gs_abi_version(void) { return GSPLAT_ABI_VERSION; }
@@ -885,7 +942,13 @@
     c->segBaseWanted = c->fast16 && N > 0;
     c->segBaseDone = false;
     c->fwdPairNow = c->fast16 && blend_forward_v2_pair_decide(c);
+    const float* const sixPtr[6] = {xyz, features_dc, features_rest, scales, rotation, opacity};
+    bool takeNext = N > 0 && c->capN >= N && next_view_matches(c, N, K, sixPtr, cp, radii);
+    if (c->nextView.accept && !takeNext) c->nextView.refused++;
+    c->nextView.accept = false;
+    c->nextView.ready = false;
     int rc = bin_with_capacity(c, N, reserved, !c->fast16, [&]() {
+        if (takeNext) { takeNext = false; return adopt_next_view(c, N); }
         return launch_projection_fused_forward(c, N, K, xyz, features_dc, features_rest, scales, rotation, opacity, cp,
                                                radii);
     });
@@ -1443,8 +1506,47 @@
     if (const int rc = blend_backward_of_forward(c, cot_color, cot_depth, cot_alpha, c->absgrad, c->adamGate)) return rc;
     c->fwd.consumed = true;
     AbsgradScope noNorm(c);
+    GsNextView& nv = c->nextView;
+    const bool next = nv.enabled && nv.armed && next_view_step_is_plain(c, params_base);
+    nv.armed = false;
+    nv.ready = false;
+    if (next) {
+        if (const int rc = ensure_next_view_ws(c)) return rc;
+        nv.N = N; nv.K = K;
+        nv.ptr[0] = c->fwd.xyz; nv.ptr[1] = c->fwd.fdc; nv.ptr[2] = c->fwd.frest; nv.ptr[3] = c->fwd.scales; nv.ptr[4] = c->fwd.rot;
+        nv.ptr[5] = c->fwd.opacity;
+        nv.flags = next_view_flags(c, N, &nv.pieces);
+        GsStageTimer t(c, GS_STAGE_PROJ_BWD);
+        if (const int rc = launch_projection_fused_backward_adam_next(c, params_base, m_base, v_base, lr, beta1, beta2, eps, grad_scale))
+            return rc;
+        nv.ready = true;
+        nv.written++;
+        return GS_OK;
+    }
     GsStageTimer t(c, GS_STAGE_PROJ_BWD);
     return launch_projection_fused_backward_adam(c, params_base, m_base, v_base, lr, beta1, beta2, eps, grad_scale);
+}
+
+int gs_set_next_view(gs_ctx* c, const gs_camera* cam)
+{
+    if (!c) return GS_ERR_INVALID_ARG;
+    c->nextView.armed = cam != nullptr;
+    if (cam) c->nextView.cam = make_cam(cam, c->W, c->H);
+    return GS_OK;
+}
+
+int gs_accept_next_view(gs_ctx* c)
+{
+    if (!c) return GS_ERR_INVALID_ARG;
+    c->nextView.accept = true;
+    return GS_OK;
+}
+
+int gs_next_view_stats(gs_ctx* c, uint32_t out[4])
+{
+    if (!c || !out) return GS_ERR_INVALID_ARG;
+    out[0] = c->nextView.written; out[1] = c->nextView.accepted; out[2] = c->nextView.refused; out[3] = (uint32_t)c->nextView.enabled;
+    return GS_OK;
 }
 
 int gs_render_backward_dp_begin(gs_ctx* c, const float* cot_color, const float* cot_depth, const float* cot_alpha,
@@ -1813,6 +1915,8 @@
     case GS_TUNE_TRIM_RECTS:
         if (value < 0 || value > 2) return fail(c, GS_ERR_INVALID_ARG, "gs_ctx_set_tuning: trim rects is 0 (the reference's squares), 1 (cut by the ellipse's box) or 2 (and into four row groups)");
         c->trimRects = value != 0; c->rowGroups = value == 2; return GS_OK;
+    case GS_TUNE_NEXT_VIEW:
+        c->nextView.enabled = value != 0; c->nextView.armed = c->nextView.ready = c->nextView.accept = false; return GS_OK;
     case GS_TUNE_FWD_TRACE_BUFFER:
         c->fwdTrace = reinterpret_cast<unsigned long long*>((uintptr_t)value); return GS_OK;
     default:
diff --git a/gaussiansplattingmlx_amd/csrc/gs_ctx.h b/gaussiansplattingmlx_amd/csrc/gs_ctx.h
--- a/gaussiansplattingmlx_amd/csrc/gs_ctx.h
+++ b/gaussiansplattingmlx_amd/csrc/gs_ctx.h
@@ -101,6 +101,25 @@
     const uint32_t* superCut = nullptr;
     int superW = 0;
     uint32_t* dropPerBlock = nullptr;
+};
+struct GsNextView {
+    int enabled = 1;
+    bool armed = false;
+    bool ready = false;
+    bool accept = false;
+    gs::CamParams cam;
+    int N = 0, K = 0, flags = 0;
+    bool pieces = false;
+    const float* ptr[6] = {nullptr, nullptr, nullptr, nullptr, nullptr, nullptr};
+    int cap = 0;
+    float* packed12 = nullptr;
+    ushort4* tileRect = nullptr;
+    uint4* tilePieces = nullptr;
+    uint32_t* tilesTouched = nullptr;
+    uint32_t* depthKey = nullptr;
+    uint32_t* depthVal = nullptr;
+    uint32_t* visPerBlock = nullptr;
+    uint32_t written = 0, accepted = 0, refused = 0;
 };
 struct GsRealGeom {
     int tileW = 16, tileH = 16, gridW = 0, gridH = 0, T = 0, tileBits = 1;
@@ -154,6 +173,7 @@
     uint32_t* bucketStart = nullptr;
     int colourRiders = 1;
     GsRiderState rider;
+    GsNextView nextView;
     int riderShare[GS_RIDE_HOSTS] = {200, 500, 300};
     int splitterSort = 1;
     int nbCap = 0;
@@ -382,6 +402,10 @@
                                      bool emitColorCot = false);
 int launch_projection_fused_backward_adam(gs_ctx* c, const float* pBase, float* mBase, float* vBase, const float lr[6], float b1,
                                           float b2, float eps, float gscale);
+int launch_projection_fused_backward_adam_next(gs_ctx* c, const float* pBase, float* mBase, float* vBase, const float lr[6], float b1,
+                                               float b2, float eps, float gscale);
+bool next_view_step_is_plain(const gs_ctx* c, const float* pBase);
+int next_view_flags(const gs_ctx* c, int N, bool* pieces);
 int launch_vis_mask(gs_ctx* c, int N, const float* radii);
 bool depth_sort_takes_splitters(const gs_ctx* c, int N);
 int launch_pose_camera(gs_ctx* c, const gs::CamParams& host, const float* delta);
diff --git a/gaussiansplattingmlx_amd/csrc/gs_proj_fwd_kernel.h b/gaussiansplattingmlx_amd/csrc/gs_proj_fwd_kernel.h
--- a/gaussiansplattingmlx_amd/csrc/gs_proj_fwd_kernel.h
+++ b/gaussiansplattingmlx_amd/csrc/gs_proj_fwd_kernel.h
@@ -160,3 +160,72 @@
     if (cc.superCut && threadIdx.x == 0) cc.dropPerBlock[blockIdx.x] = sDropped;
     if (SELF) colour_rider_wave(self, blockIdx.x * (PROJ_FUSED_THREADS / 64) + wv, shLds + wv * 64 * GS_RIDER_ROW, lane, (int)myTouched);
 }
+
+struct NextViewOut {
+    CamParams cam;
+    int tileW, tileH, gridW, gridH, flags;
+    float* packed12;
+    ushort4* tileRect;
+    uint4* tilePieces;
+    uint32_t* tilesTouched;
+    uint32_t* depthKey;
+    uint32_t* depthVal;
+    uint32_t* visPerBlock;
+};
+
+__device__ __forceinline__ bool proj_next_view_lane(const NextViewOut& nx, int p, int degree, const float (&sp)[14],
+                                                    const float* __restrict__ rest)
+{
+    const CamParams& cam = nx.cam;
+    const int noKeyForUntouched = nx.flags & 1;
+    const bool trimRects = (nx.flags & 2) && nx.tileW == 16 && nx.tileH == 16;
+    const float m[3] = {sp[0], sp[1], sp[2]};
+    const float s[3] = {expf(sp[3]), expf(sp[4]), expf(sp[5])};
+    const float r0 = sp[6], r1 = sp[7], r2 = sp[8], r3 = sp[9];
+    const float den = sqrtf(r0 * r0 + r1 * r1 + r2 * r2 + r3 * r3) + 1e-8f;
+    const float q[4] = {r0 / den, r1 / den, r2 / den, r3 / den};
+    const float opacity = 1.0f / (1.0f + expf(-sp[10]));
+    ProjOut o;
+    project_geometry<false>(m, s, q, cam, o);
+    if (GS_DEGENERATE_INVISIBLE && !(o.cov2d[0] * o.cov2d[3] - o.cov2d[1] * o.cov2d[2] > 0.0f)) o.radius = 0.0f;
+
+    uint32_t touched = 0;
+    ushort4 tr = make_ushort4(0, 0, 0, 0);
+    uint32_t pc[4] = {0u, 0u, 0u, 0u};
+    if (o.radius > 0.0f) {
+        int x0, y0, x1, y1;
+        if (trimRects)
+            block_rect_of_splat(o.rect, o.sx, o.sy, o.cov2d[0], o.cov2d[3], 1, 1, 16, 16, nx.gridW, nx.gridH, (int)cam.W, (int)cam.H,
+                                x0, y0, x1, y1);
+        else
+            tile_rect(o.rect[0], o.rect[1], o.rect[2], o.rect[3], nx.tileW, nx.tileH, nx.gridW, nx.gridH, x0, y0, x1, y1);
+        touched = (uint32_t)((x1 - x0) * (y1 - y0));
+        if (trimRects && nx.tilePieces && touched)
+            touched = rect_row_groups4(o.sx, o.sy, o.cov2d[0], o.cov2d[1], o.cov2d[3], x0, y0, x1, y1, (int)cam.H, pc);
+        tr = make_ushort4((unsigned short)x0, (unsigned short)y0, (unsigned short)x1, (unsigned short)y1);
+    }
+    float c0 = 0.f, c1 = 0.f, c2 = 0.f;
+    uint32_t gate = 0u;
+    if (touched) {
+        const float x = m[0] - cam.cam[0], y = m[1] - cam.cam[1], z = m[2] - cam.cam[2];
+        sh_foreach(degree, x, y, z, [&](int k, float b, float, float, float) {
+            if (k == 0) { c0 = b * sp[11]; c1 = b * sp[12]; c2 = b * sp[13]; }
+            else {
+                const float* r = rest + (k - 1) * 3;
+                c0 += b * r[0]; c1 += b * r[1]; c2 += b * r[2];
+            }
+        });
+        c0 += 0.5f; c1 += 0.5f; c2 += 0.5f;
+        gate = colour_gate(c0, c1, c2);
+    }
+    float4* out = reinterpret_cast<float4*>(nx.packed12 + (size_t)p * 12);
+    out[0] = make_float4(o.sx, o.sy, o.conic[0], o.conic[1]);
+    out[1] = make_float4(o.conic[2], o.conic[3], c0, c1);
+    out[2] = make_float4(c2, opacity, o.depth, __uint_as_float(gate));
+    nx.tileRect[p] = tr;
+    if (trimRects && nx.tilePieces) nx.tilePieces[p] = make_uint4(pc[0], pc[1], pc[2], pc[3]);
+    nx.tilesTouched[p] = touched;
+    nx.depthKey[p] = (touched || !noKeyForUntouched) ? __float_as_uint(o.depth) : GS_SORT_NO_KEY;
+    nx.depthVal[p] = (uint32_t)p;
+    return o.radius > 0.0f;
+}
diff --git a/gaussiansplattingmlx_amd/csrc/projection.hip b/gaussiansplattingmlx_amd/csrc/projection.hip
--- a/gaussiansplattingmlx_amd/csrc/projection.hip
+++ b/gaussiansplattingmlx_amd/csrc/projection.hip
@@ -409,16 +409,20 @@
     return v;
 }
 
-template <int MODE, bool POSE, bool AA = false, bool MCMC = false, bool F3D = false, bool SPARSE = false, bool FISHEYE = false>
+template <int MODE, bool POSE, bool AA = false, bool MCMC = false, bool F3D = false, bool SPARSE = false, bool FISHEYE = false,
+          bool NEXT = false>
 __device__ __forceinline__ void proj_bwd_fused_body(
     int N, int K, int degree, const CamParams& cam, const float* xyz, const float* fdc,
     const float* frest, const float* scalesRaw, const float* rotRaw,
     const float* opacityRaw, const float* __restrict__ gradAcc16, float* gXyz,
     float* gFdc, float* gFrest, float* gScales, float* gRot,
     float* gOpacity, float* __restrict__ gradNormAccum, AdamFuse adam, float* __restrict__ posePartials,
-    McmcFuse mc = McmcFuse{}, const float* __restrict__ filter3d = nullptr, const unsigned char* __restrict__ visMask = nullptr)
+    McmcFuse mc = McmcFuse{}, const float* __restrict__ filter3d = nullptr, const unsigned char* __restrict__ visMask = nullptr,
+    const NextViewOut* nx = nullptr)
 {
     constexpr bool EMIT_MG = MODE == 1, ADAM = MODE == 2;
+    static_assert(!NEXT || (ADAM && !POSE && !AA && !MCMC && !F3D && !SPARSE && !FISHEYE), "the next view rides in the plain Adam form only");
+    float nsp[NEXT ? 14 : 1];
     extern __shared__ float shLds[];
     const uint32_t gateWord = ADAM ? *adam.gate : 0u;
     const int p = blockIdx.x * PROJ_FUSED_THREADS + threadIdx.x;
@@ -612,12 +616,30 @@
             *reinterpret_cast<V4*>(adam.vBase + o) = V4{sv_[6], sv_[7], sv_[8], sv_[9]};
         }
         { const size_t o = small_off(10); pB[o] = sp[10]; adam.mBase[o] = sm_[10]; adam.vBase[o] = sv_[10]; }
+        if constexpr (NEXT) {
+#pragma unroll
+            for (int i = 0; i < 14; i++) nsp[i] = sp[i];
+        }
+    }
+    if constexpr (NEXT) {
+        if (!smallOn) {
+            const float sp[14] = {m[0], m[1], m[2], sr[0], sr[1], sr[2], rr[0], rr[1], rr[2], rr[3], opr, d0v[0], d0v[1], d0v[2]};
+#pragma unroll
+            for (int i = 0; i < 14; i++) nsp[i] = sp[i];
+        }
     }
     }
     if (MODE == 0 && rows > 0 && L > 0) sh_rows_out(myRows, gFrest + (size_t)row0 * L, rows, L, lane);
     if (ADAM && !gateWord && rows > 0 && L > 0) {
         if (kept) adam_rows_kept<SPARSE>(adam, frest, row0, total4, L, myRows, lane, adam.lr[2], keptRows, visBits);
         else adam_rows<SPARSE>(adam, frest, row0, rows, L, myRows, lane, adam.lr[2], visBits);
+    }
+    if constexpr (NEXT) {
+        if (kept) sh_rows_to_lds4(myRows, total4, L, 0, lane, keptRows);
+        bool visible = false;
+        if (p < N) visible = proj_next_view_lane(*nx, p, degree, nsp, myRows + lane * (L + 1));
+        const int nvis = __syncthreads_count(visible);
+        if (threadIdx.x == 0) nx->visPerBlock[blockIdx.x] = (uint32_t)nvis;
     }
     if constexpr (POSE) {
         float* out = posePartials + 16 * ((size_t)blockIdx.x * (PROJ_FUSED_THREADS / 64) + wv);
@@ -664,6 +686,14 @@
                                                            a.rotRaw, a.opacityRaw, a.gradAcc16, a.gXyz, a.gFdc, a.gFrest, a.gScales,
                                                            a.gRot, a.gOpacity, a.gradNormAccum, a.adam, a.posePartials, a.mc, a.filter3d,
                                                            a.visMask);
+}
+
+__global__ __launch_bounds__(PROJ_FUSED_THREADS) void proj_bwd_fused_next_kernel(ProjBwdArgs a, NextViewOut nx)
+{
+    proj_bwd_fused_body<2, false, false, false, false, false, false, true>(a.N, a.K, a.degree, a.cam, a.xyz, a.fdc, a.frest, a.scalesRaw,
+                                                                          a.rotRaw, a.opacityRaw, a.gradAcc16, a.gXyz, a.gFdc, a.gFrest,
+                                                                          a.gScales, a.gRot, a.gOpacity, a.gradNormAccum, a.adam,
+                                                                          a.posePartials, a.mc, a.filter3d, a.visMask, &nx);
 }
 
 __global__ __launch_bounds__(256) void vis_mask_kernel(int N, const float* __restrict__ radii, unsigned char* __restrict__ mask)
@@ -1048,7 +1078,7 @@
 }
 
 struct ProjBwdGrads { float *xyz, *fdc, *frest, *scales, *rot, *opacity; };
-static int launch_proj_bwd_fused(gs_ctx* c, int mode, const ProjBwdGrads& g, const AdamFuse& adam)
+static int launch_proj_bwd_fused(gs_ctx* c, int mode, const ProjBwdGrads& g, const AdamFuse& adam, const NextViewOut* next = nullptr)
 {
     const int N = c->fwd.N, K = c->fwd.K;
     if (N == 0) return c->fwd.poseDelta && mode != 1 ? launch_pose_grad(c, 0) : GS_OK;
@@ -1070,6 +1100,12 @@
     a.filter3d = c->fwd.filter3d;
     a.visMask = c->visMask;
     const size_t lds = sizeof(float) * (PROJ_FUSED_THREADS / 64) * 64 * ((K - 1) * 3 + 1);
+    if (next) {
+        hipLaunchKernelGGL(proj_bwd_fused_next_kernel, dim3(gs_div_up(N, PROJ_FUSED_THREADS)), dim3(PROJ_FUSED_THREADS), lds, c->stream, a,
+                           *next);
+        GS_HIP_CHECK(c, hipGetLastError());
+        return GS_OK;
+    }
     const int rc = with_flags(
         [&](auto ADAM, auto EMIT_MG, auto POSE, auto AA, auto MCMC, auto F3D, auto SPARSE, auto FISHEYE) {
             constexpr int MODE = ADAM ? 2 : EMIT_MG ? 1 : 0;
@@ -1105,6 +1141,37 @@
     a.b1 = b1; a.b2 = b2; a.eps = eps; a.gscale = gscale;
     a.gate = c->adamGate;
     return launch_proj_bwd_fused(c, 2, ProjBwdGrads{}, a);
+}
+
+bool next_view_step_is_plain(const gs_ctx* c, const float* pBase)
+{
+    const auto& f = c->fwd;
+    return c->fast16 && f.N > 0 && f.K == GS_RIDER_K && !c->virt.nbx && !f.poseDelta && !c->poseDelta && !f.antialias && !c->antialias &&
+           !f.fisheye && !c->fisheye && !f.filter3d && !c->filter3d && !c->mcmcOn && !c->sparseAdam && !c->adcGradSum &&
+           (((size_t)(f.frest - pBase)) & 3) == 0;
+}
+
+int next_view_flags(const gs_ctx* c, int N, bool* pieces)
+{
+    *pieces = c->trimRects && c->rowGroups && !c->virt.nbx && c->tileW == 16 && c->tileH == 16 && c->tilePieces != nullptr;
+    return (gs_small_depth_sort(N) ? 1 : 0) | (c->trimRects ? 2 : 0);
+}
+
+int launch_projection_fused_backward_adam_next(gs_ctx* c, const float* pBase, float* mBase, float* vBase, const float lr[6], float b1,
+                                               float b2, float eps, float gscale)
+{
+    AdamFuse a = {};
+    a.pBase = pBase; a.mBase = mBase; a.vBase = vBase;
+    for (int i = 0; i < 6; i++) a.lr[i] = lr[i];
+    a.b1 = b1; a.b2 = b2; a.eps = eps; a.gscale = gscale;
+    a.gate = c->adamGate;
+    const GsNextView& v = c->nextView;
+    NextViewOut nx;
+    nx.cam = v.cam;
+    nx.tileW = c->tileW; nx.tileH = c->tileH; nx.gridW = c->gridW; nx.gridH = c->gridH; nx.flags = v.flags;
+    nx.packed12 = v.packed12; nx.tileRect = v.tileRect; nx.tilePieces = v.pieces ? v.tilePieces : nullptr;
+    nx.tilesTouched = v.tilesTouched; nx.depthKey = v.depthKey; nx.depthVal = v.depthVal; nx.visPerBlock = v.visPerBlock;
+    return launch_proj_bwd_fused(c, 2, ProjBwdGrads{}, a, &nx);
 }
 
 static long long cc_block_floats(const gs_ctx* c, int N) { return c->ccBlockFloats > 0 ? c->ccBlockFloats : 3LL * N; }
diff --git a/gaussiansplattingmlx_amd/next_view.py b/gaussiansplattingmlx_amd/next_view.py
--- /dev/null
+++ b/gaussiansplattingmlx_amd/next_view.py
@@ -0,0 +1,52 @@
+from __future__ import annotations
+
+
+class ViewSuccessor:
+
+    def __init__(self):
+        self._after = {}
+        self._camera = {}
+        self._last = None
+
+    def observe(self, key, camera=None):
+        if key is None:
+            self._last = None
+            return
+        if camera is not None:
+            self._camera[key] = camera
+        if self._last is not None:
+            self._after[self._last] = key
+        self._last = key
+
+    def guess_key(self, key):
+        return None if key is None else self._after.get(key)
+
+    def guess(self, key):
+        nxt = self.guess_key(key)
+        return None if nxt is None else self._camera.get(nxt)
+
+    def forget(self):
+        self._after.clear()
+        self._camera.clear()
+        self._last = None
+
+
+def events_due(it: int, *, densify: bool, densify_interval: int, mcmc=None, adc=None, contrib_prune=None, filter_3d: bool = False,
+               filter3d_interval: int = 0) -> bool:
+    if densify and densify_interval > 0 and it % densify_interval == 0:
+        return True
+    if mcmc is not None and mcmc.is_event(it):
+        return True
+    if adc is not None and (adc.is_event(it) or adc.is_reset(it)):
+        return True
+    if contrib_prune is not None and contrib_prune.is_event(it):
+        return True
+    if filter_3d and filter3d_interval > 0 and (it + 1) % filter3d_interval == 0:
+        return True
+    return False
+
+
+def step_arms_next_view(*, enabled: bool, single_device: bool, fuse_adam: bool, views_per_rank: int, plain_strategy: bool,
+                        pose_opt: bool, filter_3d: bool, sparse_adam: bool, antialiased: bool, fisheye: bool, event_due: bool) -> bool:
+    return bool(enabled and single_device and fuse_adam and views_per_rank == 1 and plain_strategy and not pose_opt and
+                not filter_3d and not sparse_adam and not antialiased and not fisheye and not event_due)
diff --git a/gaussiansplattingmlx_amd/renderer.py b/gaussiansplattingmlx_amd/renderer.py
--- a/gaussiansplattingmlx_amd/renderer.py
+++ b/gaussiansplattingmlx_amd/renderer.py
@@ -10,6 +10,7 @@
 
 from . import _lib, loss_mask
 from ._lib import GsplatError
+from .next_view import ViewSuccessor
 
 TILE_SIZE_H_W = namedtuple("TILE_SIZE_H_W", ["w", "h"])
 RenderResult = namedtuple("RenderResult", ["render", "depth", "alpha", "visiility_filter", "radii"])
@@ -98,6 +99,7 @@
         self._exposure = (None, None)
         self._bilateral = (None, None)
         self._loss_mask = None
+        self.viewSuccessor = ViewSuccessor()
         if antialiased:
             self.setAntialiased(True)
 
@@ -144,10 +146,10 @@
                    colour_riders=_lib.TUNE_COLOUR_RIDERS, fwd_queues=_lib.TUNE_FWD_QUEUES, fwd_four_waves=_lib.TUNE_FWD_FOUR_WAVES,
                    fwd_fold_test_scale=_lib.TUNE_FWD_FOLD_TEST_SCALE, poison_checkpoints=_lib.TUNE_POISON_CHECKPOINTS,
                    render_only=_lib.TUNE_RENDER_ONLY, fwd_pair=_lib.TUNE_FWD_PAIR, fwd_slow_slot=_lib.TUNE_FWD_SLOW_SLOT,
-                   trim_rects=_lib.TUNE_TRIM_RECTS)
+                   trim_rects=_lib.TUNE_TRIM_RECTS, next_view=_lib.TUNE_NEXT_VIEW)
     _TUNING_DEFAULTS = dict(fwd_waves_per_simd=4, bwd_waves_per_cu=16, fwd_quadrants=1, op_fwd_ppl=1, op_bwd_ppl=1,
                             fwd_trace_buffer=0, depth_gradient=1, wide_tile_sort=1, host_overflow_errors=1, splitter_depth_sort=1,
-                            colour_riders=1, fwd_queues=8, fwd_four_waves=-1, fwd_fold_test_scale=1000, poison_checkpoints=0, render_only=0, fwd_pair=-1, fwd_slow_slot=3, trim_rects=2)
+                            colour_riders=1, fwd_queues=8, fwd_four_waves=-1, fwd_fold_test_scale=1000, poison_checkpoints=0, render_only=0, fwd_pair=-1, fwd_slow_slot=3, trim_rects=2, next_view=1)
 
     def setTuning(self, **knobs):
         for k, v in knobs.items():
@@ -349,8 +351,22 @@
                                             camera.imageWidth, camera.imageHeight, means3d, shs, opacity, scales,
                                             rotations)
 
+    def setNextView(self, camera=None):
+        if camera is None:
+            self._check(self.lib.gs_set_next_view(self.ctx, None))
+            return
+        cam = camera if isinstance(camera, _lib.gs_camera) else self._camera(
+            camera.worldViewTransform, camera.projectionMatrix, camera.cameraCenter, camera.FoVx, camera.FoVy,
+            camera.focalX, camera.focalY)
+        self._check(self.lib.gs_set_next_view(self.ctx, C.byref(cam)))
+
+    def nextViewStats(self) -> dict:
+        s = (C.c_uint32 * 4)()
+        self._check(self.lib.gs_next_view_stats(self.ctx, s))
+        return dict(written=s[0], accepted=s[1], refused=s[2], enabled=bool(s[3]))
+
     def renderForward(self, params: dict, camera, want_radii: bool = False, viewKey=None, depthCuts: bool = True,
-                      wantDepth: bool = True):
+                      wantDepth: bool = True, acceptNextView: bool = False):
         cam = camera if isinstance(camera, _lib.gs_camera) else self._camera(
             camera.worldViewTransform, camera.projectionMatrix, camera.cameraCenter, camera.FoVx, camera.FoVy,
             camera.focalX, camera.focalY)
@@ -384,6 +400,9 @@
         self._cut_view = viewKey if use else None
         self._hinted_view = viewKey if buf is not None else None
         self._check(self.lib.gs_set_depth_cuts(self.ctx, 1 if use else 0))
+        self.viewSuccessor.observe(viewKey, camera)
+        if acceptNextView:
+            self._check(self.lib.gs_accept_next_view(self.ctx))
         self._check(self.lib.gs_render_forward(self.ctx, N, K, _p(p["xyz"]), _p(p["features_dc"]),
                                                _p(p["features_rest"]), _p(p["scales"]), _p(p["rotation"]),
                                                _p(p["opacity"]), C.byref(cam), _p(color),
diff --git a/gaussiansplattingmlx_amd/trainer.py b/gaussiansplattingmlx_amd/trainer.py
--- a/gaussiansplattingmlx_amd/trainer.py
+++ b/gaussiansplattingmlx_amd/trainer.py
@@ -7,6 +7,7 @@
 import torch
 
 from ._lib import GS_ERR_REPLICA_MISMATCH, GsplatError
+from .next_view import events_due, step_arms_next_view
 from .renderer import GaussianRenderer, _p
 
 GS_ERR_WORKSPACE_OVERFLOW = 3
@@ -165,6 +166,7 @@
         N = int(params["xyz"].shape[0])
         self._pbuf = [None, None]
         self._cur = 0
+        self.version = 0
         self._gbuf = self._mbuf = self._vbuf = None
         self._mspare = self._vspare = None
         self._staged = None
@@ -205,6 +207,7 @@
     def _layout(self, N: int, capacity: int, pads=("arena", "grad", "m", "v"), stride=None):
         stride = N if stride is None else int(stride)
         floats = self._offsets(max(capacity, stride))[1]
+        self.version += 1
         self.capacity = capacity
         self.N = N
         self.stride = stride
@@ -555,6 +558,9 @@
         self._committed_params = None
         self.overflowRecoveries = 0
         self._checked_views = set()
+        self.nextView = True
+        self._nextCamera = None
+        self._nextViewFor = None
         self._exchange = (process_group is not None or dp_bootstrap is not None) and (self.world > 1 or exchange_when_single)
         self._native = self._exchange and exchange_impl == "native"
         self._dp = self._exchange or self.viewsPerRank > 1
@@ -1277,7 +1283,8 @@
                                 counts, version, source, self.viewsPerRank)
 
     def trainStep(self, camera, targetRGB, stepCameras=None, viewKey=None, targetAlpha=None, lossMask=None, targetDepth=None,
-                  depthMask=None, depthAlign=(1.0, 0.0)):
+                  depthMask=None, depthAlign=(1.0, 0.0), nextCamera=None):
+        self._nextCamera = nextCamera
         if getattr(camera, "model", "pinhole") == "fisheye":
             for on, name in ((self.pose_opt, "pose_opt"), (self.filter_3d, "filter_3d")):
                 if on:
@@ -1502,7 +1509,10 @@
     def _forwardAndLoss(self, camera, targetRGB, viewKey, lossOut):
         r, m = self.gaussRender, self.model
         wd = self._depthStep is not None
-        res = r._measure("train.forward", lambda: r.renderForward(m.getParams(), camera, viewKey=viewKey, wantDepth=wd))
+        accept = self._nextViewFor == (m.version, self.iteration)
+        self._nextViewFor = None
+        res = r._measure("train.forward", lambda: r.renderForward(m.getParams(), camera, viewKey=viewKey, wantDepth=wd,
+                                                                  acceptNextView=accept))
         if viewKey is not None and viewKey not in self._checked_views:
             self._checked_views.add(viewKey)
             if self.checkOverflow():
@@ -1605,8 +1615,11 @@
                 self.addGradientAccumulation()
             fused = True
         elif not self._exchange and self.fuse_adam:
+            armed = self._armNextView(camera, viewKey)
             r._measure("bwd.fused+train.optimizer.applySingle", lambda: r.renderBackwardAdam(
                 self._cot, m.arena, m.m, m.v, getLearningRates(self.iteration, self.iterationCount), **self._depthCots()))
+            if armed:
+                self._nextViewFor = (m.version, self.iteration + 1)
             if self.densify:
                 self.addGradientAccumulation()
             fused = True
@@ -1677,6 +1690,28 @@
             t.adam(r, int(viewKey), self.iteration, self.iterationCount)
         return self._finishIteration()
 
+    def _eventsDue(self, it: int) -> bool:
+        return events_due(it, densify=bool(self.densify), densify_interval=self.split_and_prune_per_iteration, mcmc=self.mcmc,
+                          adc=self.adc, contrib_prune=self.contribPrune, filter_3d=self.filter_3d,
+                          filter3d_interval=getattr(self, "filter3dInterval", 0))
+
+    def _armNextView(self, camera, viewKey) -> bool:
+        r = self.gaussRender
+        nxt, self._nextCamera = self._nextCamera, None
+        if not step_arms_next_view(enabled=self.nextView and r.getTuning("next_view") != 0, single_device=not self._exchange and not self._native,
+                                   fuse_adam=bool(self.fuse_adam), views_per_rank=self.viewsPerRank,
+                                   plain_strategy=self.mcmc is None and self.adc is None, pose_opt=self.pose_opt,
+                                   filter_3d=self.filter_3d, sparse_adam=bool(self.sparse_adam) or getattr(r, "_sparse_adam", False),
+                                   antialiased=bool(getattr(r, "_antialiased", False)),
+                                   fisheye=getattr(camera, "model", "pinhole") == "fisheye", event_due=self._eventsDue(self.iteration)):
+            return False
+        if nxt is None:
+            nxt = r.viewSuccessor.guess(viewKey)
+        if nxt is None or getattr(nxt, "model", "pinhole") != "pinhole":
+            return False
+        r.setNextView(nxt)
+        return True
+
     def _finishIteration(self):
         r, m = self.gaussRender, self.model
         it = self.iteration
diff --git a/include/gsplat.h b/include/gsplat.h
--- a/include/gsplat.h
+++ b/include/gsplat.h
@@ -106,6 +106,10 @@
 int gs_render_backward_adam(gs_ctx* ctx, const float* cot_color, const float* cot_depth, const float* cot_alpha,
                             float* params_base, float* m_base, float* v_base, long long n_arena, const float lr[6],
                             float beta1, float beta2, float eps, float grad_scale);
+
+int gs_set_next_view(gs_ctx* ctx, const gs_camera* cam );
+int gs_accept_next_view(gs_ctx* ctx);
+int gs_next_view_stats(gs_ctx* ctx, uint32_t out[4] );
 
 int gs_render_contrib(gs_ctx* ctx, float* max_w , float* sum_w );
 
@@ -396,6 +400,7 @@
     GS_TUNE_FWD_PAIR = 16,
     GS_TUNE_FWD_SLOW_SLOT = 17,
     GS_TUNE_TRIM_RECTS = 18,
+    GS_TUNE_NEXT_VIEW = 19,
     GS_TUNE_POISON_CHECKPOINTS = 14,
     GS_TUNE_DEPTH_GRADIENT = 6
 } gs_tuning;
```
